# DoHoonKim8/halo2-lasso

Measured on AMD Instinct MI355X. Metric: lasso_prove_time_ms, lower is better.
Workload: dtype u256 (BN254 Fr/Fq, 8x u32 Montgomery); 1 GPU; 2^24 AND Lasso lookup (32-bit operands, 4 chunks of 8+8 bits); lookups_per_proof=16777216, pcs=multilinear KZG (BN254), proof_bytes=64256, parallelism=1 GPU

## Files before the change

### bindings/rust/src/sys.rs

```rust
#![allow(non_camel_case_types, dead_code)]
use halo2_curves::bn256::{Fr, G1Affine, G2Affine};
use std::os::raw::{c_char, c_int, c_void};

pub type lh_status = c_int;
pub const LH_OK: lh_status = 0;
pub const LH_ERR_INVALID_SUMCHECK: lh_status = -1;
pub const LH_ERR_INVALID_PCS_PARAM: lh_status = -2;
pub const LH_ERR_INVALID_PCS_OPEN: lh_status = -3;
pub const LH_ERR_INVALID_SNARK: lh_status = -4;
pub const LH_ERR_SERIALIZATION: lh_status = -5;
pub const LH_ERR_TRANSCRIPT: lh_status = -6;
pub const LH_ERR_DEVICE: lh_status = -7;
pub const LH_ERR_ARG: lh_status = -8;

pub const LH_SC_MAX_TERMS: usize = 48;
pub const LH_SC_MAX_FACTORS: usize = 4;
pub const LH_SC_EVALUATIONS: c_int = 0;
pub const LH_SC_COEFFICIENTS: c_int = 1;
pub const LH_LASSO_MAX_CHUNKS: usize = 8;
pub const LH_LASSO_MAX_MEMORIES: usize = 16;
pub const LH_LASSO_MAX_TERMS: usize = 16;
pub const LH_RCCL_UNIQUE_ID_BYTES: usize = 128;

#[repr(C)] pub struct lh_ctx { _p: [u8; 0] }
// ... 71 lines not shown
    pub g_num_factors: [u8; LH_LASSO_MAX_TERMS],
    pub g_factor: [[u8; LH_SC_MAX_FACTORS]; LH_LASSO_MAX_TERMS],
}

#[repr(C)]
pub struct lh_comm {
    pub rank: c_int,
    pub size: c_int,
    pub user: *mut c_void,
    pub all_gather: Option<unsafe extern "C" fn(*mut c_void, *const c_void, *mut c_void, usize) -> c_int>,
    pub all_gather_device: Option<unsafe extern "C" fn(*mut c_void, *const c_void, *mut c_void, usize, *mut c_void) -> c_int>,
}

#[repr(C)]
pub struct lh_hp_lookup { pub inputs: *const lh_expr, pub tables: *const lh_expr, pub width: usize }
#[repr(C)] #[derive(Clone, Copy)]
pub struct lh_hp_lasso_lookup {
    pub table: lh_lasso_table,
    pub output_poly: usize,
    pub chunk_polys: [usize; LH_LASSO_MAX_CHUNKS],
}
#[repr(C)]
pub struct lh_hp_param {
    pub num_vars: usize,
    pub num_instance_polys: usize,
    pub num_instances: *const usize,
    pub num_preprocess_polys: usize,
    pub d_preprocess_polys: *const *const c_void,
    pub num_witness_polys: usize,
    pub num_challenges: usize,
    pub num_lookups: usize,
    pub lookups: *const lh_hp_lookup,
    pub num_permutation_polys: usize,
    pub permutation_poly_index: *const usize,
    pub d_permutation_polys: *const *const c_void,
    pub num_permutation_z_polys: usize,
    pub expression: lh_expr,
    pub num_lasso_lookups: usize,
    pub lasso_lookups: *const lh_hp_lasso_lookup,
}
#[repr(C)]
pub struct lh_hp_vparam {
    pub num_vars: usize,
    pub num_instance_polys: usize,
    pub num_instances: *const usize,
    pub num_witness_polys: usize,
    pub num_challenges: usize,
    pub num_lookups: usize,
    pub num_permutation_z_polys: usize,
    pub expression: lh_expr,
    pub num_preprocess_polys: usize,
    pub preprocess_comms: *const G1Affine,
    pub num_permutation_polys: usize,
    pub permutation_comms: *const G1Affine,
    pub num_lasso_lookups: usize,
    pub lasso_lookups: *const lh_hp_lasso_lookup,
}
#[repr(C)]
pub struct lh_hp_circuit {
    pub user: *mut c_void,
    pub synthesize: Option<unsafe extern "C" fn(*mut c_void, usize, *const Fr, usize, *mut *const c_void, usize) -> c_int>,
}

#[repr(C)]
#[derive(Clone, Copy, Debug, Default)]
pub struct lh_lasso_route {
    pub open_small_depth: u32,
    pub open_small_passes: u32,
    pub eq_factored_rounds: u32,
    pub standard_rounds: u32,
    pub rw_leaf_rounds: u32,
    pub resident_tails: u32,
    pub resident_rounds: u32,
    pub packed_ts_pairs: u32,
    pub derived_commitments: u32,
    pub sorted_dim_reuse: u32,
    pub sharded_rounds: u32,
    pub shard_exchanges: u32,
    pub window_table_jobs: u32,
    pub open_precommit: u32,
    pub resident_layers: u32,
    pub pp_folds: u32,
    pub msm_half_batches: u32,
    pub reserved: [u32; 7],
}

extern "C" {
    pub fn lh_last_error() -> *const c_char;
    pub fn lh_version() -> *const c_char;
    pub fn lh_ctx_create(device_id: c_int, out: *mut *mut lh_ctx) -> lh_status;
    pub fn lh_ctx_destroy(ctx: *mut lh_ctx);
    pub fn lh_ctx_sync(ctx: *mut lh_ctx) -> lh_status;
    pub fn lh_ctx_stream(ctx: *mut lh_ctx) -> *mut c_void;
    pub fn lh_alloc(ctx: *mut lh_ctx, bytes: usize, d_out: *mut *mut c_void) -> lh_status;
    pub fn lh_free(ctx: *mut lh_ctx, d_ptr: *mut c_void) -> lh_status;
    pub fn lh_upload(ctx: *mut lh_ctx, d_dst: *mut c_void, src: *const c_void, bytes: usize) -> lh_status;
    pub fn lh_download(ctx: *mut lh_ctx, dst: *mut c_void, d_src: *const c_void, bytes: usize) -> lh_status;
    pub fn lh_fr_from_u64(ctx: *mut lh_ctx, d_in: *const u64, n: usize, d_out: *mut Fr) -> lh_status;
    pub fn lh_fr_from_u32(ctx: *mut lh_ctx, d_in: *const u32, n: usize, d_out: *mut Fr) -> lh_status;
    pub fn lh_fr_batch_invert(ctx: *mut lh_ctx, d_in: *const Fr, n: usize, d_out: *mut Fr) -> lh_status;
    pub fn lh_fix_var(ctx: *mut lh_ctx, d_in: *const Fr, n_in: usize, x: *const Fr, d_out: *mut Fr) -> lh_status;
    pub fn lh_eq_xy(ctx: *mut lh_ctx, y: *const Fr, num_vars: usize, d_out: *mut Fr) -> lh_status;
    pub fn lh_evaluate(ctx: *mut lh_ctx, d_polys: *const *const Fr, num_polys: usize, num_vars: usize,
                       point: *const Fr, out_evals: *mut Fr) -> lh_status;
    pub fn lh_lincomb(ctx: *mut lh_ctx, d_polys: *const *const Fr, w: *const Fr, num_polys: usize, n: usize,
                      d_out: *mut Fr) -> lh_status;
    pub fn lh_sumcheck_prove(ctx: *mut lh_ctx, prover_kind: c_int, num_vars: usize, expr: *const lh_sop,
                             d_polys: *const *const Fr, num_polys: usize, ys: *const Fr, num_ys: usize,
                             sum: *const Fr, t: *mut lh_transcript, out_challenges: *mut Fr, out_evals: *mut Fr) -> lh_status;
    pub fn lh_sumcheck_prove_expr(ctx: *mut lh_ctx, num_vars: usize, expr: *const lh_expr, d_polys: *const *const Fr,
                                  num_polys: usize, challenges: *const Fr, num_challenges: usize, ys: *const Fr,
                                  num_ys: usize, sum: *const Fr, t: *mut lh_transcript, out_challenges: *mut Fr,
                                  out_evals: *mut Fr) -> lh_status;
    pub fn lh_sumcheck_verify(prover_kind: c_int, num_vars: usize, degree: usize, sum: *const Fr,
                              t: *mut lh_transcript, out_eval: *mut Fr, out_x: *mut Fr) -> lh_status;
    pub fn lh_gkr_fractional_prove(ctx: *mut lh_ctx, num_batching: usize, num_vars: usize,
                                   claimed_p_0s: *const *const Fr, claimed_q_0s: *const *const Fr,
                                   d_ps: *const *const Fr, d_qs: *const *const Fr, t: *mut lh_transcript,
                                   out_p_xs: *mut Fr, out_q_xs: *mut Fr, out_x: *mut Fr) -> lh_status;
    pub fn lh_msm(ctx: *mut lh_ctx, d_scalars: *const Fr, d_bases: *const G1Affine, n: usize, out: *mut G1Affine) -> lh_status;
    pub fn lh_msm_u32(ctx: *mut lh_ctx, d_scalars: *const u32, d_bases: *const G1Affine, n: usize, out: *mut G1Affine) -> lh_status;
    pub fn lh_srs_upload(ctx: *mut lh_ctx, eqs_flat: *const G1Affine, num_vars: usize, out: *mut *mut lh_srs) -> lh_status;
    pub fn lh_srs_num_vars(srs: *const lh_srs) -> usize;
    pub fn lh_srs_free(ctx: *mut lh_ctx, srs: *mut lh_srs);
    pub fn lh_mkzg_batch_commit(ctx: *mut lh_ctx, srs: *const lh_srs, d_polys: *const *const Fr, num_polys: usize,
                                num_vars: usize, out_comms: *mut G1Affine) -> lh_status;
    pub fn lh_mkzg_open(ctx: *mut lh_ctx, srs: *const lh_srs, d_poly: *const Fr, num_vars: usize, point: *const Fr,
                        t: *mut lh_transcript, out_eval: *mut Fr) -> lh_status;
    pub fn lh_mkzg_batch_open(ctx: *mut lh_ctx, srs: *const lh_srs, num_vars: usize, d_polys: *const *const Fr,
                              num_polys: usize, points: *const Fr, num_points: usize, evals: *const lh_evaluation,
                              num_evals: usize, t: *mut lh_transcript) -> lh_status;
    pub fn lh_mkzg_vp_new(g1: *const G1Affine, g2: *const G2Affine, ss: *const G2Affine, num_vars: usize,
                          out: *mut *mut lh_mkzg_vp) -> lh_status;
    pub fn lh_mkzg_vp_free(vp: *mut lh_mkzg_vp);
    pub fn lh_mkzg_verify(vp: *const lh_mkzg_vp, comm: *const G1Affine, point: *const Fr, num_vars: usize,
                          eval: *const Fr, t: *mut lh_transcript) -> lh_status;
    pub fn lh_mkzg_batch_verify(vp: *const lh_mkzg_vp, num_vars: usize, comms: *const G1Affine, num_comms: usize,
                                points: *const Fr, num_points: usize, evals: *const lh_evaluation, num_evals: usize,
                                t: *mut lh_transcript) -> lh_status;
    pub fn lh_lasso_prove(ctx: *mut lh_ctx, srs: *const lh_srs, table: *const lh_lasso_table, num_vars: usize,
                          d_dims: *const *const u32, t: *mut lh_transcript) -> lh_status;
    pub fn lh_lasso_verify(vp: *const lh_mkzg_vp, table: *const lh_lasso_table, num_vars: usize,
                           t: *mut lh_transcript) -> lh_status;
    pub fn lh_ctx_set_comm(ctx: *mut lh_ctx, comm: *const lh_comm, shard_bit: usize) -> lh_status;
    pub fn lh_rccl_unique_id(out: *mut u8) -> lh_status;
    pub fn lh_ctx_set_comm_rccl(ctx: *mut lh_ctx, rank: c_int, size: c_int, unique_id: *const u8, shard_bit: usize) -> lh_status;
    pub fn lh_ctx_set_comm_loopback(ctx: *mut lh_ctx, rank: c_int, size: c_int, shard_bit: usize) -> lh_status;
    pub fn lh_ctx_comm_stats(ctx: *mut lh_ctx, out: *mut u64) -> lh_status;
    pub fn lh_ctx_comm_phase_stats(ctx: *mut lh_ctx, out: *mut u64, reset: c_int) -> lh_status;
    pub fn lh_ctx_memory_stats(ctx: *mut lh_ctx, out: *mut u64) -> lh_status;
    pub fn lh_ctx_host_cpus(ctx: *mut lh_ctx, bus_id: *mut c_char, bus_id_cap: usize, cpulist: *mut c_char, cpulist_cap: usize) -> lh_status;
    pub fn lh_shard_extract(ctx: *mut lh_ctx, d_global: *const c_void, n_local: usize, shard_bit: usize, rho: usize,
                            rank: usize, elem_bytes: usize, d_local: *mut c_void) -> lh_status;
    pub fn lh_ctx_set_option(ctx: *mut lh_ctx, name: *const c_char, value: i64) -> lh_status;
    pub fn lh_ctx_get_option(ctx: *mut lh_ctx, name: *const c_char, out: *mut i64) -> lh_status;
    pub fn lh_lasso_last_route(ctx: *mut lh_ctx, out: *mut lh_lasso_route) -> lh_status;
    pub fn lh_lasso_prove_sharded(ctx: *mut lh_ctx, srs: *const lh_srs, table: *const lh_lasso_table, num_vars: usize,
                                  d_dims_local: *const *const u32, t: *mut lh_transcript) -> lh_status;
    pub fn lh_hyperplonk_prove(ctx: *mut lh_ctx, srs: *const lh_srs, pp: *const lh_hp_param,
                               instances: *const *const Fr, d_witness_polys: *const *const Fr,
                               t: *mut lh_transcript) -> lh_status;
    pub fn lh_hyperplonk_prove_sharded(ctx: *mut lh_ctx, srs: *const lh_srs, pp: *const lh_hp_param,
                                       instances: *const *const Fr, d_witness_polys_local: *const *const Fr,
                                       t: *mut lh_transcript) -> lh_status;
    pub fn lh_hyperplonk_prove_phases(ctx: *mut lh_ctx, srs: *const lh_srs, pp: *const lh_hp_param, num_phases: usize,
                                      num_witness_polys: *const usize, num_challenges: *const usize,
                                      instances: *const *const Fr, circuit: *const lh_hp_circuit,
// ... 135 lines not shown
```

### halo2-lasso_amd/__init__.py

```python
import ctypes as C

from . import _ffi
from ._ffi import (lh_fr, lh_g1, lh_sop, lh_evaluation, lh_lasso_table, lh_transcript,
                   LH_SC_EVALUATIONS, LH_SC_COEFFICIENTS)

R_MOD = 0x30644E72E131A029B85045B68181585D2833E84879B9709143E1F593F0000001
Q_MOD = 0x30644E72E131A029B85045B68181585D97816A916871CA8D3C208C16D87CFD47
_MONT = 1 << 256
_MONT_INV_R = pow(_MONT, -1, R_MOD)
_MONT_INV_Q = pow(_MONT, -1, Q_MOD)

SUBTABLE_IDENTITY, SUBTABLE_AND, SUBTABLE_XOR = 0, 1, 2


class Error(Exception):
    code = None


class InvalidSumcheck(Error):
    code = _ffi.LH_ERR_INVALID_SUMCHECK


class InvalidPcsParam(Error):
    code = _ffi.LH_ERR_INVALID_PCS_PARAM
# ... 1360 lines not shown
                return _ffi.LH_ERR_ARG
            C.memmove(recv, out, len(out))
            return 0
        except Exception:
            return _ffi.LH_ERR_DEVICE
    comm = _ffi.lh_comm()
    comm.rank, comm.size, comm.user = rank, size, None
    comm.all_gather = _ffi._AG_CB(cb)
    ctx._comm_keepalive = (comm, cb)
    _check(ctx.lib.lh_ctx_set_comm(ctx.h, C.byref(comm), shard_bit))


def rccl_unique_id():
    buf = C.create_string_buffer(_ffi.LH_RCCL_UNIQUE_ID_BYTES)
    _check(_ffi.load().lh_rccl_unique_id(buf))
    return buf.raw


def attach_comm_rccl(ctx, rank, size, unique_id, shard_bit):
    if len(unique_id) != _ffi.LH_RCCL_UNIQUE_ID_BYTES:
        raise ArgumentError("unique id must be %d bytes" % _ffi.LH_RCCL_UNIQUE_ID_BYTES)
    _check(ctx.lib.lh_ctx_set_comm_rccl(ctx.h, rank, size, unique_id, shard_bit))


def comm_stats(ctx):
    out = (C.c_uint64 * 2)()
    _check(ctx.lib.lh_ctx_comm_stats(ctx.h, out))
    return {"device": int(out[0]), "host": int(out[1])}


def comm_phase_stats(ctx, reset=False):
    out = (C.c_uint64 * 16)()
    _check(ctx.lib.lh_ctx_comm_phase_stats(ctx.h, out, 1 if reset else 0))
    names = ["witness", "commit", "surge", "leaves", "gkr", "evals", "open", "outside"]
    return {nm: {"collectives": int(out[2 * i]), "bytes": int(out[2 * i + 1])} for i, nm in enumerate(names) if out[2 * i]}


def memory_stats(ctx):
    out = (C.c_uint64 * 4)()
    _check(ctx.lib.lh_ctx_memory_stats(ctx.h, out))
    return {"arena_high_water_bytes": int(out[0]), "arena_reserved_bytes": int(out[1]), "device_free_bytes": int(out[2]),
            "device_total_bytes": int(out[3])}


def attach_comm_loopback(ctx, rank, size, shard_bit):
    _check(ctx.lib.lh_ctx_set_comm_loopback(ctx.h, rank, size, shard_bit))


def detach_comm(ctx):
    _check(ctx.lib.lh_ctx_set_comm(ctx.h, None, 0))
    ctx._comm_keepalive = None


def shard_of(column, rank, size, shard_bit):
    rho = size.bit_length() - 1
    n = len(column)
    return column.reshape(n >> (shard_bit + rho), size, 1 << shard_bit)[:, rank, :].reshape(-1).copy()


def shard_poly(poly, rank, size, shard_bit):
    rho = size.bit_length() - 1
    n_local = (1 << poly.num_vars) >> rho
    out = poly.ctx.alloc(32 * n_local)
    _check(poly.ctx.lib.lh_shard_extract(poly.ctx.h, poly.ptr, n_local, shard_bit, rho, rank, 32, out.ptr))
    return MultilinearPolynomial(poly.ctx, out, poly.num_vars - rho)


def lasso_prove_sharded(pp, table, num_vars, dims_local, transcript):
    if len(dims_local) != table.c:
        raise ArgumentError("expected %d dim columns" % table.c)
    t = table.to_c()
    _check(pp.ctx.lib.lh_lasso_prove_sharded(pp.ctx.h, pp.h, C.byref(t), num_vars, _ptr_array(dims_local), transcript.p))


def lasso_last_timing(ctx):
    out = (C.c_double * _ffi.LH_LASSO_NUM_PHASES)()
    _check(ctx.lib.lh_lasso_last_timing(ctx.h, out))
    names = ["witness", "commit", "surge", "leaves", "gkr", "evals", "open_n", "open_l", "total"]
    return dict(zip(names, list(out)))


ROUTE_FIELDS = ["open_small_depth", "open_small_passes", "eq_factored_rounds", "standard_rounds", "rw_leaf_rounds",
                "resident_tails", "resident_rounds", "packed_ts_pairs", "derived_commitments", "sorted_dim_reuse",
                "sharded_rounds", "shard_exchanges", "window_table_jobs", "open_precommit", "resident_layers", "pp_folds", "msm_half_batches"]


def lasso_last_route(ctx):
    out = (C.c_uint32 * 24)()
    _check(ctx.lib.lh_lasso_last_route(ctx.h, out))
    return dict(zip(ROUTE_FIELDS, [int(v) for v in out]))


def set_option(ctx, name, value):
    _check(ctx.lib.lh_ctx_set_option(ctx.h, name.encode(), int(value)))


def get_option(ctx, name):
    out = C.c_int64(0)
    _check(ctx.lib.lh_ctx_get_option(ctx.h, name.encode(), C.byref(out)))
    return int(out.value)


def profile_enable(ctx, on=True):
    _check(ctx.lib.lh_profile_enable(ctx.h, int(on)))


def profile_read(ctx):
    n = C.c_size_t()
    _check(ctx.lib.lh_profile_read(ctx.h, None, 0, C.byref(n)))
    arr = (_ffi.lh_prof_rec * max(n.value, 1))()
    _check(ctx.lib.lh_profile_read(ctx.h, arr, n.value, C.byref(n)))
    return [dict(name=r.name.decode(), ms=r.ms, bytes=r.bytes, muls=r.muls, items=r.items) for r in arr[:n.value]]


from . import expression
```

### halo2-lasso_amd/csrc/dev.cpp

```cpp
#include <string.h>
#include <stdlib.h>
#include <ctype.h>
#include <errno.h>
#include <sched.h>
#include <atomic>
#include <condition_variable>
#include <mutex>
#include <thread>
#include <functional>
#include <memory>
#include <emmintrin.h>
#include <hip/hip_ext.h>
#include <vector>
#include <chrono>
#include "dev.hpp"

namespace lh {

static thread_local std::string g_last_error;
void set_last_error(const char* msg) { g_last_error = msg ? msg : ""; }
const char* get_last_error() { return g_last_error.c_str(); }

Arena::~Arena() {
  for (auto& b : blocks_) (void)hipFree(b.p);
}

void* Arena::alloc(size_t bytes) {
  bytes = (bytes + 255) & ~(size_t)255;
  if (bytes == 0) bytes = 256;
  return alloc_raw(bytes);
}
void* Arena::alloc_raw(size_t bytes) {
  while (true) {
    if (!blocks_.empty()) {
      Block& b = blocks_[cur_];
      if (b.used + bytes <= b.size) {
        void* p = b.p + b.used;
        b.used += bytes;
        size_t tot = 0;
        for (size_t i = 0; i <= cur_; i++) tot += blocks_[i].used;
        if (tot > high_) high_ = tot;
        return p;
      }
      if (cur_ + 1 < blocks_.size()) {
        cur_++;
        blocks_[cur_].used = 0;
        continue;
      }
    }
    size_t want = blocks_.empty() ? ((size_t)64 << 20) : blocks_.back().size * 2;
    if (want < bytes) want = bytes;
    void* p = nullptr;
    LH_HIP(hipMalloc(&p, want));
    blocks_.push_back(Block{(char*)p, want, 0});
    cur_ = blocks_.size() - 1;
  }
}

void Arena::release(Mark m) {
  if (blocks_.empty()) return;
  for (size_t i = m.block + 1; i < blocks_.size(); i++) blocks_[i].used = 0;
  cur_ = m.block;
  blocks_[cur_].used = m.used;
}

void Ctx::opt_in_lds(const void* fn, int bytes) {
  for (const void* f : lds_opted)
    if (f == fn) return;
  LH_HIP(hipFuncSetAttribute(fn, hipFuncAttributeMaxDynamicSharedMemorySize, bytes));
  lds_opted.push_back(fn);
}

static const struct {
  const char* name;
  int64_t Options::*field;
  int64_t lo, hi;
} OPTION_TABLE[] = {
    {"open_small_min_vars", &Options::open_small_min_vars, 0, 64}, {"open_small_depth", &Options::open_small_depth, 0, 2},
    {"sc_eq_factoring", &Options::sc_eq_factoring, 0, 1},          {"lasso_pack_ts", &Options::lasso_pack_ts, 0, 1},
    {"sc_tail", &Options::sc_tail, 0, 1},                          {"sc_tail_max_len", &Options::sc_tail_max_len, 0, (int64_t)1 << 20},
    {"shard_exchange_log", &Options::shard_exchange_log, 0, 40},   {"msm_window_tables", &Options::msm_window_tables, 0, 40},
    {"open_precommit", &Options::open_precommit, 0, 64},           {"gkr_resident", &Options::gkr_resident, 0, 1},
    {"sc_pp_fold", &Options::sc_pp_fold, 0, 2},                    {"msm_half_batches", &Options::msm_half_batches, 0, 1},
    {"comm_round", &Options::comm_round, 0, 2},
};

int64_t* Options::find(const char* name) {
  if (!name) return nullptr;
  for (const auto& o : OPTION_TABLE)
    if (strcmp(o.name, name) == 0) return &(this->*o.field);
  return nullptr;
}
bool Options::in_range(const char* name, int64_t value) {
  if (!name) return false;
  for (const auto& o : OPTION_TABLE)
    if (strcmp(o.name, name) == 0) return value >= o.lo && value <= o.hi;
  return false;
}

static bool env_number(const char* name, bool real, double lo, double hi, double& out, std::atomic<bool>* said = nullptr) {
  const char* e = getenv(name);
  if (!e || !*e) return false;
  char* end = nullptr;
  errno = 0;
  const double v = real ? strtod(e, &end) : (double)strtoll(e, &end, 10);
  if (end != e && *end == 0 && errno == 0 && v >= lo && v <= hi) {
    out = v;
    return true;
  }
  if (!said || !said->exchange(true))
    fprintf(stderr, "[lasso-hip] %s=%s is outside [%lld, %lld]: ignored\n", name, e, (long long)lo, (long long)hi);
  return false;
}

Options::Options() {
  for (const auto& o : OPTION_TABLE) {
    std::string env = "LH_";
    for (const char* p = o.name; *p; p++) env.push_back((char)toupper((unsigned char)*p));
    double v;
    if (!env_number(env.c_str(), false, (double)o.lo, (double)o.hi, v)) continue;
    this->*o.field = (int64_t)v;
    if (o.field == &Options::open_small_min_vars) open_small_min_vars_forced = true;
  }
}

enum KnobKind { INT, REAL, WORD, PATH };
static constexpr struct KnobRow {
  const char* env;
  KnobKind kind;
  double dflt, lo, hi;
  bool live;
  const char* word;
} KNOB_TABLE[] = {
    {"LH_SC_TAIL_G", INT, 0, 0, 1024},
    {"LH_MSM_C_OFF", INT, 4, -32, 32},
    {"LH_MSM_C_MAX", INT, 17, 1, 31},
    {"LH_MSM_K2", INT, 4, 2, 64},
    {"LH_MSM_SEG", INT, 0, 0, 256},
    {"LH_MSM_SLAB_LOG", INT, 16, 0, 31},
    {"LH_MSM_TREE_MAX", INT, 262144, 0, 1 << 30},
    {"LH_MSM_QUAD_MAX", INT, 262144, 0, 1 << 30},
    {"LH_MSM_TWO_LEVEL", INT, 1, 0, 1},
    {"LH_MSM_HALF_MIN_LOG", INT, 24, 0, 63},
    {"LH_MSM_HALF_COVER", INT, 12, 0, 1 << 20},
    {"LH_EXPR_MONOMIALS", INT, 0, 0, 1},
    {"LH_EXPR_JIT_MIN_VARS", INT, 16, 0, 64},
    {"LH_EXPR_EF_MIN_VARS", INT, 14, 2, 64},
    {"LH_FIN_LANES_MIN_BYTES", REAL, 0, -1, 1e18},
    {"LH_SC_U32", INT, 1, 0, 1}, {"LH_OPEN_U32_ROUNDS", INT, 1, 0, 1}, {"LH_OPEN_FOLD_COLS", INT, 1, 0, 1},
    {"LH_HOST_THREADS", INT, 48, 0, 4096},
    {"LH_JIT_CACHE", INT, 1, 0, 1}, {"LH_JIT_CACHE_DIR", PATH, 0, 0, 0},
    {"LH_EXPR_JIT", INT, 1, 0, 1},
    {"LH_SC_TAIL_TIMEOUT_MS", REAL, 2000, 0, 1e7, true}, {"LH_GKR_START_TIMEOUT_MS", REAL, 25, 0, 1e7, true},
    {"LH_COMM_WAIT_TIMEOUT_MS", INT, 30000, 1, 1e9}, {"LH_COMM_A2A", WORD, 0, 0, 1, false, "allgather"},
    {"LH_COMM_PROBE", INT, 1, 0, 1},
    {"LH_HOST_TRACE", INT, 0, 0, 1, true}, {"LH_SC_TAIL_TRACE", INT, 0, 0, 1}, {"LH_GKR_TRACE", INT, 0, 0, 1},
    {"LH_SC_DEBUG", INT, 0, 0, 1}, {"LH_MSM_DEBUG", INT, 0, 0, 1}, {"LH_HP_DEBUG", INT, 0, 0, 1}, {"LH_COMM_DEBUG", INT, 0, 0, 1},
    {"LH_OPEN_SMALL_CHECK", INT, 0, 0, 1},
    {"LH_COMM_A2A_SELF", INT, 0, 0, 1}, {"LH_COMM_PROBE_FAIL", INT, 0, 0, 1}, {"LH_SHARDED_COUNTERS_MIN_R", INT, 2, 1, 1 << 20},
};
static_assert(sizeof(KNOB_TABLE) / sizeof(KNOB_TABLE[0]) == (size_t)Knob::COUNT, "KNOB_TABLE: one row per Knob");

static double knob_read(const KnobRow& r, std::atomic<bool>* said) {
  double v = r.dflt;
  if (r.kind != WORD) {
    env_number(r.env, r.kind == REAL, r.lo, r.hi, v, said);
  } else if (const char* e = getenv(r.env)) {
// ... 417 lines not shown
```

### halo2-lasso_amd/csrc/dev.hpp

```cpp
#pragma once
#include <hip/hip_runtime_api.h>
#include <stdint.h>
#include <stdarg.h>
#include <stdio.h>
#include <functional>
#include <string>
#include <vector>
#include <utility>
#include <stdexcept>

#include "../../include/lasso_hip.h"
#include "ec.cuh"

namespace lh {

struct Error : std::exception {
  int code;
  std::string msg;
  Error(int c, std::string m) : code(c), msg(std::move(m)) {}
  const char* what() const noexcept override { return msg.c_str(); }
};

void set_last_error(const char* msg);

// ... 1 lines not shown
  do {                                                                                     \
    hipError_t e_ = (expr);                                                                \
    if (e_ != hipSuccess)                                                                  \
      throw ::lh::Error(LH_ERR_DEVICE, std::string(#expr) + ": " + hipGetErrorString(e_)); \
  } while (0)

#define LH_REQUIRE(cond, code, text) \
  do {                               \
    if (!(cond)) throw ::lh::Error((code), (text)); \
  } while (0)

class Arena {
 public:
  struct Mark {
    size_t block, used;
  };
  ~Arena();
  void* alloc(size_t bytes);
  void* alloc_raw(size_t bytes);
  template <class T>
  T* alloc_n(size_t n) {
    return (T*)alloc(n * sizeof(T));
  }
  Mark mark() const { return {cur_, blocks_.empty() ? 0 : blocks_[cur_].used}; }
  void release(Mark m);
  size_t high_water() const { return high_; }
  size_t reserved() const {
    size_t t = 0;
    for (const Block& b : blocks_) t += b.size;
    return t;
  }

 private:
  struct Block {
    char* p;
    size_t size, used;
  };
  std::vector<Block> blocks_;
  size_t cur_ = 0, high_ = 0;
};

struct ArenaScope {
  Arena& a;
  Arena::Mark m;
  explicit ArenaScope(Arena& a_) : a(a_), m(a_.mark()) {}
  ~ArenaScope() { a.release(m); }
};

struct ProfRec {
  char name[40];
  double ms;
  double bytes;
  double muls;
  double items;
};

struct ScFinishArgs {
  uint32_t* ticket;
  uint32_t last_ticket;
  Fr* out_host;
  uint32_t* flag;
  uint32_t seq;
  uint64_t* wide;
  uint32_t tag;
  uint64_t* lanes;
};
constexpr uint32_t FIN_LANE_SUMS = 65536;
constexpr unsigned SC_LANE_TAG_SHIFT = 40;

struct Options {
  int64_t open_small_min_vars = 21;
  bool open_small_min_vars_forced = false;
  int64_t open_small_depth = 0;
  int64_t sc_eq_factoring = 1;
  int64_t lasso_pack_ts = 1;
  int64_t sc_tail = 1;
  int64_t sc_tail_max_len = 8192;
  int64_t shard_exchange_log = 19;
  int64_t open_precommit = 1;
  int64_t msm_window_tables = 0;
  int64_t sc_pp_fold = 1;
  int64_t msm_half_batches = 1;
  int64_t gkr_resident = 1;
  int64_t comm_round = 0;
  Options();
  int64_t* find(const char* name);
  static bool in_range(const char* name, int64_t value);
};

enum class Knob {
  SC_TAIL_G, MSM_C_OFF, MSM_C_MAX, MSM_K2, MSM_SEG, MSM_SLAB_LOG, MSM_TREE_MAX, MSM_QUAD_MAX, MSM_TWO_LEVEL, MSM_HALF_MIN_LOG,
  MSM_HALF_COVER, EXPR_MONOMIALS, EXPR_JIT_MIN_VARS, EXPR_EF_MIN_VARS,
  FIN_LANES_MIN_BYTES, SC_U32, OPEN_U32_ROUNDS, OPEN_FOLD_COLS,
  HOST_THREADS, JIT_CACHE, JIT_CACHE_DIR, EXPR_JIT, SC_TAIL_TIMEOUT_MS, GKR_START_TIMEOUT_MS, COMM_WAIT_TIMEOUT_MS, COMM_A2A,
  COMM_PROBE,
  HOST_TRACE, SC_TAIL_TRACE, GKR_TRACE, SC_DEBUG, MSM_DEBUG, HP_DEBUG, COMM_DEBUG, OPEN_SMALL_CHECK,
  COMM_A2A_SELF, COMM_PROBE_FAIL, SHARDED_COUNTERS_MIN_R,
  COUNT
};
double knob(Knob k);
const char* knob_text(Knob k);
struct RouteStats {
  uint32_t v[LH_LASSO_ROUTE_WORDS] = {0};
  enum { OPEN_DEPTH, OPEN_PASSES, EF_ROUNDS, STD_ROUNDS, RW_ROUNDS, TAILS, TAIL_ROUNDS, PACKED_TS, DERIVED, SORTED_REUSE,
         SHARDED_ROUNDS, SHARD_EXCHANGES, WIN_TABLE_JOBS, OPEN_PRECOMMIT, RESIDENT_LAYERS, PP_FOLDS, MSM_HALF_BATCHES };
};

class HostWorker {
 public:
  HostWorker();
  ~HostWorker();
  void submit(std::function<void()> fn);
  void wait();
 private:
  struct Impl;
  Impl* impl_;
};

struct OpenPrecommit;
struct Ctx {
  Options opt;
  RouteStats route;
  int device = 0;
  hipStream_t stream = nullptr;
  Arena arena;
  void* pinned = nullptr;
  size_t pinned_bytes = 0;
  int num_cus = 256;
  int wall_clock_khz = 100000;
  double lasso_ms[LH_LASSO_NUM_PHASES] = {0};
  lh_comm comm = {0, 1, nullptr, nullptr, nullptr};
  bool has_comm = false;
  bool comm_loopback = false;
  size_t shard_bit = 0;
  bool shard_active = false;
  void* rccl_comm = nullptr;
  void* comm_stage = nullptr;
  size_t comm_stage_bytes = 0;
  uint64_t comm_stats[2] = {0, 0};
  uint64_t comm_phase_stats[8][2] = {};
  int comm_phase = 7;
  Fr* sc_redirect = nullptr;
  uint64_t* sc_wide = nullptr;
  uint32_t sc_tag = 0;
  uint32_t sc_tag_seq = 0;
  uint64_t* lanes_host = nullptr;
  bool comm_host_recv_ok = true;
  Fr* round_out(Fr* out_host) const { return sc_redirect ? sc_redirect : out_host; }
  void wait_round(uint32_t seq) {
    if (!sc_redirect) wait_flag(seq);
  }
  uint64_t* tail_trace = nullptr;
  std::vector<std::pair<const char*, double>> host_stamps;
  bool host_trace_on = false;
  void host_stamp(const char* tag);
  void host_stamps_print();
  struct EqHalfEntry {
    std::vector<uint8_t> key;
    const Fr* table;
    bool sharded = false;
  };
  std::vector<EqHalfEntry> eq_half_cache;
  bool prof = false;
  std::vector<ProfRec> prof_recs;
  bool live = false;
  struct LiveRec {
    ProfRec rec;
    hipEvent_t e0, e1;
    uint32_t batch;
  };
  std::vector<LiveRec> live_recs;
  std::vector<hipEvent_t> live_pool;
  uint32_t live_batch = 0;
  hipEvent_t live_event();
  void live_resolve(std::vector<ProfRec>& out);
  bool is_helper = false;
  Ctx* helper = nullptr;
  lh_ctx* helper_handle = nullptr;
  OpenPrecommit* precommit = nullptr;
  HostWorker* worker = nullptr;
  hipEvent_t handoff_ev = nullptr;
  hipEvent_t phase_ev[LH_LASSO_NUM_PHASES] = {};
  bool phase_ev_pending = false;
  void phase_times_resolve();
  hipEvent_t prof_ev[2] = {nullptr, nullptr};
  void* pin(size_t bytes);
  void* stage = nullptr;
  size_t stage_bytes = 0;
// ... 126 lines not shown
void k_lincomb_bind2(Ctx&, const uint32_t* const* cols, const size_t* lens, const Fr* w, size_t count, const Fr& r0, const Fr& r1,
                     const Fr* eq_level, size_t size, Fr* out, Fr* out_host);
void k_sc_round_u32_bind2(Ctx&, const uint32_t* col, const Fr* eq_level, const Fr& r0, const Fr& r1, size_t size, Fr* out,
                          Fr* out_host);
void k_lincomb_mixed(Ctx&, const Fr* const* fr, const Fr* wfr, size_t num_fr, const uint32_t* const* sm,
                     const size_t* sm_len, const Fr* wsm, size_t num_sm, size_t n, Fr* out);
void k_tree_up(Ctx&, const Fr* in, size_t half, Fr* out);
void k_tree_up_multi(Ctx&, const Fr* const* in, Fr* const* out, size_t count, size_t half);
void k_tree_tops(Ctx&, const Fr* const* in, Fr* const* out, const int* H, size_t count);
void k_frac_up(Ctx&, const Fr* p, const Fr* q, size_t half, Fr* vp, Fr* vq);
void k_quotient_step(Ctx&, const Fr* rem, size_t half, const Fr& x, Fr* q, Fr* rem_out);
void k_lasso_rw_leaves(Ctx&, const uint32_t* dim, const uint32_t* e, const uint32_t* ts, size_t n,
                       const Fr& gamma, const Fr& gamma2, const Fr& tau, Fr* rs, Fr* ws);
void k_lasso_rw_leaves_up(Ctx&, const uint32_t* dim, const uint32_t* e, const uint32_t* ts, size_t n, const Fr& gamma,
                          const Fr& gamma2, const Fr& tau, Fr* rs, Fr* ws, Fr* rs_up, Fr* ws_up);
void k_lasso_if_leaves(Ctx&, int subtable, uint32_t chunk_bits, const uint32_t* final_cts, size_t m,
                       const Fr& gamma, const Fr& gamma2, const Fr& tau, Fr* init, Fr* fin);
void k_or_u32(Ctx&, const uint32_t* const* cols, size_t count, size_t n, uint32_t* out_host);
void k_fill_u32(Ctx&, uint32_t* out, uint32_t value, size_t n);
void k_pack_u32(Ctx&, const uint32_t* a, const uint32_t* b, uint32_t shift, size_t n, uint32_t* out);
void k_delta_u32(Ctx&, const uint32_t* col, size_t len, size_t half, uint64_t offset, uint32_t* out_lo, uint32_t* out_hi);
void k_lasso_counters(Ctx&, const uint32_t* const* dims, size_t cc, size_t n, size_t m, uint32_t* const* read_ts,
                      uint32_t* const* final_cts, uint32_t* const* keep_sorted = nullptr, uint32_t* const* keep_index = nullptr);
void k_cs_partition(Ctx&, const uint32_t* const* dims, size_t cc, size_t n, size_t m, unsigned rho, unsigned j, unsigned hi_bits,
                    uint32_t* const* sidx, uint32_t* const* send, uint32_t* start_host, bool* bad_out);
void k_cs_rank(Ctx&, const uint32_t* const* recv, const size_t* n_recv, size_t cc, unsigned hi_bits, unsigned a_bits, size_t m_loc,
               uint32_t* const* ret, uint32_t* counts);
void k_cs_scatter(Ctx&, const uint32_t* const* back, const uint32_t* const* sidx, size_t cc, size_t n, uint32_t* const* read_ts);
void k_cs_final(Ctx&, const uint32_t* all_counts, size_t cc, size_t m, unsigned rho, size_t m_loc, uint32_t* const* final_cts);
void k_lasso_subtable_read(Ctx&, int subtable, uint32_t chunk_bits, const uint32_t* dim, size_t n, uint32_t* e);
struct LassoG {
  uint32_t num_terms;
  Fr coeff[LH_LASSO_MAX_TERMS];
  uint8_t nfac[LH_LASSO_MAX_TERMS];
  uint8_t fac[LH_LASSO_MAX_TERMS][LH_SC_MAX_FACTORS];
  const uint32_t* e[LH_LASSO_MAX_MEMORIES];
};
void k_lasso_output(Ctx&, const LassoG& g, size_t n, Fr* a);
struct LassoGSmall {
  uint32_t num_terms;
  uint32_t coeff[LH_LASSO_MAX_TERMS];
  uint8_t fac[LH_LASSO_MAX_TERMS];
  const uint32_t* e[LH_LASSO_MAX_MEMORIES];
};
void k_lasso_output_small(Ctx&, const LassoGSmall& g, size_t n, uint32_t* a);
bool k_fr_to_index(Ctx&, const Fr* in, size_t n, uint32_t bits, uint32_t* out);
bool k_fr_tables_equal(Ctx&, const Fr* a, const Fr* b, size_t n);

void rccl_unique_id(uint8_t out[LH_RCCL_UNIQUE_ID_BYTES]);
void comm_attach_rccl(Ctx&, int rank, int size, const uint8_t id[LH_RCCL_UNIQUE_ID_BYTES], size_t shard_bit);
void comm_probe_host_recv(Ctx&);
void comm_attach_loopback(Ctx&, int rank, int size, size_t shard_bit);
void comm_detach(Ctx&);
void comm_all_gather_dev(Ctx&, const void* d_send, void* d_recv, size_t bytes);
void comm_all_gather_host(Ctx&, const void* send, void* recv, size_t bytes);
void comm_all_to_all_multi(Ctx&, size_t nbuf, const void* const* d_send, const size_t* send_off, const size_t* send_cnt,
                           void* const* d_recv, const size_t* recv_off, const size_t* recv_cnt, const size_t* peer_off,
                           const void* send_base, size_t send_stride, size_t elem);
void comm_sum_publish(Ctx&, const Fr* d_part, Fr* d_scratch, size_t count, Fr* out_host, uint32_t seq);
void comm_sum_lanes(Ctx&, uint64_t* d_lanes, uint64_t* d_scratch, size_t count, Fr* out_host);
uint32_t comm_next_tag(Ctx&);
void k_loopback_allreduce_lanes(Ctx&, const uint64_t* d_in, size_t n, size_t R, uint64_t* out);

void k_shard_merge(Ctx&, const void* gathered, size_t n_local, size_t j, size_t rho, size_t elem, void* global);
void k_gather_interleave(Ctx&, const Fr* gathered, size_t count, size_t n_local, size_t R, size_t block, Fr* const* out);
void k_sum_publish(Ctx&, const Fr* all, size_t R, size_t D, Fr* out_host, uint32_t seq);
void k_shard_extract(Ctx&, const void* global, size_t n_local, size_t j, size_t rho, size_t s, size_t elem, void* local);
void k_loopback_gather(Ctx&, const void* d_send, void* d_recv, size_t bytes, size_t R);
void k_scale(Ctx&, const Fr* in, const Fr& w, size_t n, Fr* out);

constexpr int SC_MAX_TABLES = 72;
struct ScRound {
  const Fr* in[SC_MAX_TABLES];
  Fr* out[SC_MAX_TABLES];
  uint32_t num_tables;
  uint32_t num_terms;
  int32_t global_eq;
  Fr coeff[LH_SC_MAX_TERMS];
  uint8_t coeff_is_one[LH_SC_MAX_TERMS];
  uint8_t nfac[LH_SC_MAX_TERMS];
  uint8_t fac[LH_SC_MAX_TERMS][LH_SC_MAX_FACTORS];
  Fr r;
  const Fr* eq_level;
  uint8_t pp;
};
bool k_sc_round(Ctx&, const ScRound& rd, int degree, bool bind, size_t size, Fr* evals_host);
bool k_sc_round_streams(const ScRound& rd, int degree, size_t size);
void k_eq_levels(Ctx&, const Fr* in, size_t n_in, Fr* const* levels, size_t nlev);
constexpr int SC_OPEN_MAX_TERMS = 6;
struct ScOpenRound {
  const Fr* in[SC_OPEN_MAX_TERMS];
  Fr* out[SC_OPEN_MAX_TERMS];
  const Fr* eq_level[SC_OPEN_MAX_TERMS];
  uint32_t num_terms;
  Fr r;
};
void k_sc_round_open(Ctx&, const ScOpenRound& rd, bool bind, size_t size, Fr* out_host);

constexpr int SC_RW_MAX_PAIRS = 8;
struct ScRwRound {
  const Fr* l[SC_RW_MAX_PAIRS];
  const Fr* r[SC_RW_MAX_PAIRS];
  Fr* lo[SC_RW_MAX_PAIRS];
  Fr* ro[SC_RW_MAX_PAIRS];
  Fr cs[SC_RW_MAX_PAIRS], k[SC_RW_MAX_PAIRS];
  const Fr* eq_level;
  Fr rchal;
  uint32_t num_pairs;
};
void k_sc_round_rw(Ctx&, const ScRwRound& rd, bool bind, size_t size, Fr* out_host, bool fold = false);

struct TailChunk {
  uint32_t w[4];
};
struct TailMbox {
  TailChunk c[3];
  uint32_t pad[4];
};
constexpr uint32_t SC_TAIL_ABORT = 0xffffffffu;
constexpr int SC_TAIL_MAX_DEGREE = 6;
size_t k_sc_tail_capacity(const Ctx&, const ScRound& rd, int degree);
void k_sc_tail_launch(Ctx&, const ScRound& rd, int degree, size_t n0, bool first_bind, size_t num_out, uint32_t seq0,
                      TailChunk* msg_host, Fr* out_host);
void k_sc_tail_resync(Ctx&);

constexpr int GKR_MAX_TREES = 16;
constexpr int GKR_MAX_VARS = 16;
constexpr uint32_t GKR_CAP = 128;
constexpr uint32_t GKR_THREADS = 256;
constexpr uint32_t GKR_MSG_CHUNKS = 3 * (GKR_MAX_TREES + GKR_MAX_VARS);
constexpr uint32_t GKR_START_FAILED = 0xfffffffeu;
enum { GKR_F_SPLIT = 1, GKR_F_BIND = 2, GKR_F_EQ = 4, GKR_F_NOMSG = 8, GKR_F_KOFF = 16 };
struct GkrLayerDev {
  const Fr* lv[GKR_MAX_TREES];
  const Fr* rv[GKR_MAX_TREES];
  uint32_t h, B;
  uint32_t g, s_log;
  uint32_t seq;
  uint32_t flags;
  const Fr* eq_level;
  Fr r_prev;
  Fr coef[GKR_MAX_TREES];
  Fr koff[GKR_MAX_TREES];
};
bool k_gkr_resident_geometry(uint32_t h, uint32_t* g, uint32_t* s_log);
void k_gkr_resident_launch(Ctx&, const GkrLayerDev* layers, size_t num_layers, TailChunk* msg_host, Fr* out_host);

struct ExtRound {
  const Fr* in[SC_MAX_TABLES];
  Fr* out[SC_MAX_TABLES];
  uint32_t num_tables, num_terms;
  const Fr* coeff;
  const uint8_t* is_one;
  const uint32_t* off;
  const uint8_t* fac;
  const uint8_t* store;
  Fr r;
};
void k_sc_round_ext(Ctx&, const ExtRound& rd, int degree, bool bind, size_t size, Fr* evals_host);
void k_rotate_gather(Ctx&, const Fr* poly, size_t num_vars, int rot, uint32_t primitive, uint32_t x_inv, Fr* out);
void k_identity_table(Ctx&, size_t n, Fr* out);
void k_identity_table_shard(Ctx&, size_t n_local, size_t j, size_t rho, size_t rank, Fr* out);
void k_bh_order(Ctx&, size_t num_vars, uint32_t primitive, uint32_t* order, uint32_t* nth);
void k_one_hot_table(Ctx&, size_t n, size_t hot, Fr* out);
enum { PROG_ADD = 0, PROG_SUB = 1, PROG_MUL = 2, PROG_NEG = 3, PROG_MOV = 4 };
enum { PROG_REG = 0, PROG_ATOM = 1, PROG_CONST = 2, PROG_PAIR = 3 };
constexpr int PROG_MAX_REGS = 8;
struct ProgRound {
  const Fr* in[SC_MAX_TABLES];
  uint32_t num_tables, num_instrs, num_regs, result_reg;
  const uint32_t* code;
  const Fr* consts;
};
struct JitKernel;
bool jit_enabled(size_t num_vars);
std::string jit_debug_source(const uint32_t* code, size_t num_instrs, uint32_t num_regs, uint32_t result_reg, int degree);
const JitKernel* jit_sc_round(const Ctx&, const uint32_t* host_code, size_t num_instrs, uint32_t num_regs, uint32_t result_reg, int degree);
unsigned jit_blocks_per_cu(const JitKernel*);
void jit_launch(Ctx&, const JitKernel*, const ProgRound& pr, unsigned points, unsigned grid, size_t size, Fr* partials, const ScFinishArgs& fin);
void k_sc_round_prog(Ctx&, const ProgRound& pr, int points, size_t size, Fr* evals_host, const JitKernel* jit = nullptr);
constexpr int LIN_MAX_TABLES = 8;
struct LinSums {
  const Fr* t[LIN_MAX_TABLES];
  Fr coeff[LIN_MAX_TABLES];
  uint32_t count;
};
void k_lin_sums(Ctx&, const LinSums& ls, size_t size, Fr* out_host);
enum { ROWS_ATOM_POLY = 0, ROWS_ATOM_IDENTITY = 1, ROWS_ATOM_LAGRANGE = 2 };
struct RowsAtom {
// ... 109 lines not shown
```

### halo2-lasso_amd/csrc/gkr.cpp

```cpp
#include <algorithm>
#include <functional>
#include <chrono>
#include <memory>
#include <thread>
#include "host.hpp"
#include "resident_host.hpp"

namespace lh {

FracSumCheckResult prove_fractional_sum_check(Ctx& c, size_t B, size_t num_vars, const HFr* const* claimed_p_0s,
                                              const HFr* const* claimed_q_0s, const Fr* const* d_ps,
                                              const Fr* const* d_qs, Transcript& tr) {
  LH_REQUIRE(B != 0, LH_ERR_ARG, "fractional sum-check: num_batching == 0");
  LH_REQUIRE(num_vars >= 1, LH_ERR_ARG, "fractional sum-check: num_vars == 0");
  LH_REQUIRE(3 * B <= LH_SC_MAX_TERMS && 4 * B + 1 <= (size_t)SC_MAX_TABLES, LH_ERR_ARG,
             "fractional sum-check: too many fractions for one round kernel");
  ArenaScope scope(c.arena);
  std::vector<std::vector<const Fr*>> lp(num_vars), lq(num_vars);
  for (size_t b = 0; b < B; b++) {
    lp[0].push_back(d_ps[b]);
    lq[0].push_back(d_qs[b]);
  }
  for (size_t h = 1; h < num_vars; h++) {
    size_t half = (size_t)1 << (num_vars - h);
// ... 107 lines not shown
    std::vector<int> top_H(B);
    std::vector<size_t> cur_h(B);
    size_t max_h = 0;
    for (size_t b = 0; b < B; b++) {
      level[b].resize(num_vars[b]);
      level[b][num_vars[b] - 1] = d_leaves[b];
      size_t h = num_vars[b] - 1;
      if (d_level_up && d_level_up[b] && h > SMALL && (!sh.on || sh.sharded(h))) {
        level[b][h - 1] = d_level_up[b];
        h--;
      }
      cur_h[b] = h;
      max_h = std::max(max_h, h);
    }
    for (size_t h = max_h; h >= 1 && (h > SMALL || sh.sharded(h + 1)); h--) {
      std::vector<const Fr*> ins;
      std::vector<Fr*> outs;
      std::vector<size_t> who;
      const bool in_sh = sh.sharded(h + 1), out_sh = sh.sharded(h);
      const size_t half = (size_t)1 << (in_sh ? h - sh.rho : h);
      for (size_t b = 0; b < B; b++) {
        if (cur_h[b] != h) continue;
        ins.push_back(level[b][h]);
        who.push_back(b);
        cur_h[b] = h - 1;
      }
      if (ins.empty()) continue;
      if (in_sh && !out_sh) {
        Fr* block = c.arena.alloc_n<Fr>(ins.size() * half);
        std::vector<Fr*> rep(ins.size());
        for (size_t k = 0; k < ins.size(); k++) {
          outs.push_back(block + k * half);
          rep[k] = c.arena.alloc_n<Fr>((size_t)1 << h);
        }
        k_tree_up_multi(c, ins.data(), outs.data(), ins.size(), half);
        comm_gather_tables(c, block, ins.size(), half, half, rep.data());
        c.route.v[RouteStats::SHARD_EXCHANGES]++;
        for (size_t k = 0; k < ins.size(); k++) level[who[k]][h - 1] = rep[k];
      } else {
        for (size_t k = 0; k < ins.size(); k++) {
          outs.push_back(c.arena.alloc_n<Fr>(half));
          level[who[k]][h - 1] = outs.back();
        }
        k_tree_up_multi(c, ins.data(), outs.data(), ins.size(), half);
      }
    }
    for (size_t b = 0; b < B; b++) {
      const size_t h = cur_h[b];
      LH_REQUIRE(h <= SMALL && !sh.sharded(h + 1), LH_ERR_ARG, "grand product: internal level mismatch");
      Fr* tops = c.arena.alloc_n<Fr>(((size_t)2 << h));
      top_in[b] = level[b][h];
      top_out[b] = tops;
      top_H[b] = (int)h;
      for (size_t k = 0; k < h; k++) level[b][k] = tops + (((size_t)2 << k) - 2);
    }
    k_tree_tops(c, top_in.data(), top_out.data(), top_H.data(), B);
  }
  std::vector<HFr> top(2 * B);
  {
    std::vector<const Fr*> heads;
    for (size_t b = 0; b < B; b++) heads.push_back(level[b][0]);
    Fr* out = (Fr*)c.pin(2 * SC_MAX_TABLES * sizeof(Fr));
    k_gather_heads(c, heads.data(), heads.size(), 2, out);
    memcpy(top.data(), out, 2 * B * sizeof(Fr));
  }
  GrandProductResult res;
  res.roots.resize(B);
  res.claims.resize(B);
  res.points.resize(B);
  for (size_t b = 0; b < B; b++) res.roots[b] = top[2 * b] * top[2 * b + 1];
  tr.write_field_elements(res.roots);

  std::vector<HFr> claims = res.roots, y;
  HFr resident_lam;
  bool have_resident_lam = false;
  GkrResident resident(c);
  std::vector<GkrLayerDev> resident_layers;
  if (c.opt.gkr_resident && c.opt.sc_tail && c.opt.sc_eq_factoring) {
    std::vector<GkrLayerDev> layers;
    for (size_t h = 1; h < max_depth; h++) {
      GkrLayerDev L;
      memset(&L, 0, sizeof(L));
      uint32_t nb = 0;
      bool ok = !sh.sharded(h + 1) && k_gkr_resident_geometry((uint32_t)h, &L.g, &L.s_log);
      bool any_leaf = false, all_leaf = true;
      for (size_t b = 0; b < B && ok; b++) {
        if (num_vars[b] <= h) continue;
        ok = nb < (uint32_t)GKR_MAX_TREES && level[b][h] != nullptr;
        if (!ok) break;
        any_leaf = any_leaf || num_vars[b] == h + 1;
        all_leaf = all_leaf && num_vars[b] == h + 1;
        L.lv[nb++] = level[b][h];
      }
      if (ok && plus_one && any_leaf && all_leaf) ok = false;
      if (!ok || nb == 0) break;
      L.h = (uint32_t)h, L.B = nb;
      layers.push_back(L);
    }
    resident_layers.swap(layers);
  }
  if (trees_built) trees_built();
  if (!resident_layers.empty()) resident.launch(resident_layers);
  for (size_t h = 0; h < max_depth; h++) {
    std::vector<size_t> active;
    for (size_t b = 0; b < B; b++)
      if (num_vars[b] > h) active.push_back(b);
    if (h >= 1 && resident.live && h <= resident.H) {
      HFr lam = tr.squeeze_challenge();
      HFr claim = HFr::zero(), power = HFr::one();
      std::vector<HFr> coeff;
      for (size_t b : active) {
        claim += claims[b] * power;
        coeff.push_back(power);
        power *= lam;
      }
      std::vector<HFr> x, evals;
      if (resident.layer(h, coeff, y, claim, tr, x, evals)) {
        c.route.v[RouteStats::RESIDENT_LAYERS]++;
        tr.write_field_elements(evals);
        HFr mu = tr.squeeze_challenge();
        x.push_back(mu);
        y = x;
        for (size_t k = 0; k < active.size(); k++) {
          const size_t b = active[k];
          const HFr &l = evals[2 * k], &r = evals[2 * k + 1];
          claims[b] = l + mu * (r - l);
          if (num_vars[b] == h + 1) {
            res.claims[b] = claims[b];
            res.points[b] = y;
          }
        }
        continue;
      }
      resident_lam = lam, have_resident_lam = true;
    }
    const bool layer_sh = sh.sharded(h + 1);
    const size_t half = (size_t)1 << (layer_sh ? h - sh.rho : h);
    std::vector<HFr> x, evals;
    if (h == 0) {
      for (size_t b : active) {
        evals.push_back(top[2 * b]);
        evals.push_back(top[2 * b + 1]);
      }
    } else {
      HFr lam = have_resident_lam ? resident_lam : tr.squeeze_challenge();
      have_resident_lam = false;
      HFr claim = HFr::zero(), power = HFr::one();
      lh_sop expr;
      memset(&expr, 0, sizeof(expr));
      expr.global_eq = 0;
      std::vector<const Fr*> polys;
      ScOptions so;
      so.sum_is_exact = true, so.sharded = layer_sh;
      bool pairs = plus_one != nullptr && active.size() % 2 == 0 && active.size() / 2 <= (size_t)SC_RW_MAX_PAIRS;
      for (size_t k = 0; k < active.size() && pairs; k++) {
        const size_t b = active[k];
        pairs = num_vars[b] == h + 1 && (k % 2 == 0 ? !plus_one[b] : (plus_one[b] && active[k - 1] + 1 == b));
      }
      if (pairs) {
        const size_t P = active.size() / 2;
        ScRwPairs rw;
        rw.num_pairs = (uint32_t)P;
        rw.const_total = HFr::zero();
        HFr cw_sum = HFr::zero();
        bool degenerate = false;
        uint32_t t = 0;
        for (size_t i = 0; i < P; i++) {
// ... 66 lines not shown
```

### halo2-lasso_amd/csrc/host.hpp

```cpp
#pragma once
#include <string.h>
#include <functional>
#include <map>
#include <mutex>
#include <vector>
#include "dev.hpp"
#include "ff_host.hpp"

namespace lh {

const char* get_last_error();

typedef host::Fr HFr;
typedef host::G1Affine HG1;

static inline Fr dev(const HFr& f) {
  Fr r;
  memcpy(&r, &f, 32);
  return r;
}
static inline HFr hst(const Fr& f) {
  HFr r;
  memcpy(&r, &f, 32);
  return r;
// ... 48 lines not shown
  }
  void common_commitment(const HG1& p) { check(t->common_commitment(t->user, (const lh_g1*)&p)); }
  HFr read_field_element() {
    LH_REQUIRE(t->read_field_element, LH_ERR_ARG, "transcript cannot read (write-only callback table)");
    HFr f;
    check(t->read_field_element(t->user, (lh_fr*)&f));
    return f;
  }
  std::vector<HFr> read_field_elements(size_t n) {
    std::vector<HFr> v(n);
    for (auto& f : v) f = read_field_element();
    return v;
  }
  HG1 read_commitment() {
    LH_REQUIRE(t->read_commitment, LH_ERR_ARG, "transcript cannot read (write-only callback table)");
    HG1 p;
    check(t->read_commitment(t->user, (lh_g1*)&p));
    return p;
  }
  std::vector<HG1> read_commitments(size_t n) {
    std::vector<HG1> v(n);
    for (auto& p : v) p = read_commitment();
    return v;
  }
};

typedef std::function<void(size_t num_vars, const HG1* comms, size_t num_comms, const HFr* points, size_t num_points,
                           const lh_evaluation* evals, size_t num_evals, Transcript& tr)>
    PcsBatchVerify;

std::vector<HFr> host_eq_xy(const std::vector<HFr>& y);
HFr host_eq_xy_eval(const HFr* x, const HFr* y, size_t n);
std::vector<HFr> evaluate_polys(Ctx&, const Fr* const* d_polys, size_t count, size_t num_vars, const HFr* point);

struct SumCheckResult {
  std::vector<HFr> challenges;
  std::vector<HFr> evals;
  bool u32_terms_built = false;
};
struct ScRwPairs {
  uint32_t num_pairs;
  HFr cs[SC_RW_MAX_PAIRS], k[SC_RW_MAX_PAIRS];
  HFr const_total;
};
struct ScU32 {
  const uint32_t* col = nullptr;
  bool have_sums = false;
  Fr odd, s2, s3;
};
struct ScU32Terms {
  struct Poly {
    std::vector<const uint32_t*> col;
    std::vector<size_t> len;
    std::vector<Fr> w;
  };
  std::vector<Poly> polys;
};
struct ScOptions {
  bool sum_is_exact = false;
  bool sharded = false;
  const ScRwPairs* rw = nullptr;
  const ScU32* u32 = nullptr;
  const ScU32Terms* u32_terms = nullptr;
};
SumCheckResult sum_check_prove(Ctx&, int prover_kind, size_t num_vars, const lh_sop& expr, const Fr* const* d_polys,
                               size_t num_polys, const HFr* ys, size_t num_ys, const HFr& sum, Transcript& tr,
                               const ScOptions& opt = ScOptions());

const Fr* eq_half_lookup(Ctx&, const HFr* y, size_t num_vars, bool sharded = false);
const Fr* eq_half_get(Ctx&, const HFr* y, size_t num_vars, bool sharded = false);
struct EqHalfScope {
  Ctx& c;
  size_t mark;
  explicit EqHalfScope(Ctx& c_) : c(c_), mark(c_.eq_half_cache.size()) {}
  ~EqHalfScope() { c.eq_half_cache.resize(mark); }
};

typedef std::function<void(const Fr* const*, Fr* const*, const Fr&, bool, size_t, Fr*)> RoundFn;
struct EqFactoring {
  struct One {
    size_t table;
    const HFr* y;
    std::vector<const Fr*> level;
    HFr S, S_prev;
    std::vector<HFr> q;
  };
  std::vector<One> eqs;
  bool per_term = false;
  bool trusted_claim = false;
  bool untrusted = false;
  std::vector<HFr> inv_1my;
  HFr c;
  HFr add_const;
  HFr kappa = HFr::one(), lin0 = HFr::zero(), lin1 = HFr::zero();
  std::function<bool(bool bind, size_t size)> streams;
  std::function<void(const Fr* const* in, Fr* const* out, const Fr& r, bool bind, size_t size, size_t round, int points,
                     Fr* out_host)>
      round;
  std::function<bool(const std::vector<const Fr*>& cur, bool bind, const HFr& r_prev, size_t n0, size_t round, const HFr& claim,
                     Transcript& tr, SumCheckResult& res)>
      resident_tail;
};
SumCheckResult sum_check_loop(Ctx&, int prover_kind, size_t num_vars, int degree, std::vector<const Fr*> cur,
                              const std::vector<char>& used, size_t num_polys, const HFr& sum, Transcript& tr,
                              bool sharded, const RoundFn& round_fn, const ScRound* tail_rd = nullptr,
                              EqFactoring* ef = nullptr);
SumCheckResult sum_check_prove_expr(Ctx&, size_t num_vars, const lh_expr& expr, const Fr* const* d_polys,
                                    size_t num_polys, const HFr* challenges, size_t num_challenges, const HFr* ys,
                                    size_t num_ys, const HFr& sum, Transcript& tr, bool sharded = false);

std::vector<HFr> evaluate_polys(Ctx&, const Fr* const* d_polys, size_t count, size_t num_vars, const HFr* point, bool sharded);
void comm_sum_fr(Ctx&, HFr* v, size_t n);
void comm_sum_points(Ctx&, HG1* pts, size_t n);
void comm_gather_tables(Ctx&, const Fr* local_block, size_t count, size_t n_local, size_t block, Fr* const* out);
void comm_gather_concat(Ctx&, const Fr* local, size_t n_local, Fr* out);
void eq_xy_shard(Ctx&, const Shard&, const HFr* y, size_t num_vars, size_t first, Fr* out_local);

struct FracSumCheckResult {
  std::vector<HFr> p_xs, q_xs, x;
};
FracSumCheckResult prove_fractional_sum_check(Ctx&, size_t num_batching, size_t num_vars,
                                              const HFr* const* claimed_p_0s, const HFr* const* claimed_q_0s,
                                              const Fr* const* d_ps, const Fr* const* d_qs, Transcript& tr);
struct GrandProductResult {
  std::vector<HFr> roots, claims;
  std::vector<std::vector<HFr>> points;
};
GrandProductResult prove_grand_product(Ctx&, size_t num_trees, const Fr* const* d_leaves, const size_t* num_vars,
                                       Transcript& tr, const Fr* const* d_level_up = nullptr,
                                       const uint8_t* plus_one = nullptr,
                                       const std::function<void()>& trees_built = nullptr);

struct Srs {
  G1Affine* d_eqs = nullptr;
  size_t num_vars = 0;
  const G1Affine* eq(size_t k) const { return d_eqs + (((size_t)1 << k) - 1); }
  mutable std::vector<G1Affine*> shard_levels;
  mutable int shard_rank = -1;
  mutable size_t shard_R = 0, shard_j = 0;
  mutable std::map<size_t, HG1> level_sums;
  mutable std::map<size_t, HG1> shard_level_sums;
  struct WinTable {
    G1Affine* d = nullptr;
    uint32_t c = 0, W = 0;
  };
  mutable std::map<size_t, WinTable> win_tables;
};
const Srs::WinTable* srs_window_table(Ctx&, const Srs&, size_t level);
const G1Affine* srs_shard_level(Ctx&, const Srs&, size_t level);
Srs* mkzg_setup(Ctx&, const HFr* ss, size_t num_vars);
std::vector<HG1> mkzg_batch_commit(Ctx&, const Srs&, const Fr* const* d_polys, size_t num_polys, size_t num_vars);
std::vector<HG1> mkzg_batch_commit_u32(Ctx&, const Srs&, const uint32_t* const* d_polys, size_t num_polys,
                                       size_t num_vars);
struct SmallOpen;
HFr mkzg_open(Ctx&, const Srs&, const Fr* d_poly, size_t num_vars, const HFr* point, Transcript& tr,
              const SmallOpen* small = nullptr);
struct SmallLinear {
  std::vector<size_t> poly;
  std::vector<HFr> coeff;
};
struct SmallPoly {
  const uint32_t* ptr = nullptr;
  size_t len = 0;
  uint32_t bits = 0;
  const SmallLinear* linear = nullptr;
};
// ... 229 lines not shown
```

### halo2-lasso_amd/csrc/kernels_poly.hip

```cpp
#include <hip/hip_runtime.h>
#include <string.h>
#include <algorithm>
#include "dev.hpp"
#include "ff_host.hpp"
#include "reduce.cuh"
#include "resident.cuh"
#include "wide.cuh"

namespace lh {

static inline dim3 grid_for(size_t n, int block = 256, size_t cap = 4096) {
  size_t g = (n + block - 1) / block;
  if (g < 1) g = 1;
  if (g > cap) g = cap;
  return dim3((unsigned)g);
}
#define GSTRIDE(i, n) \
  for (size_t i = (size_t)blockIdx.x * blockDim.x + threadIdx.x; i < (n); i += (size_t)gridDim.x * blockDim.x)

__global__ void fr_from_u64_kernel(const uint64_t* __restrict__ in, size_t n, Fr* __restrict__ out) {
  GSTRIDE(i, n) out[i] = from_u64<FrParams>(in[i]);
}
__global__ void fr_from_u32_kernel(const uint32_t* __restrict__ in, size_t n, Fr* __restrict__ out) {
  GSTRIDE(i, n) out[i] = from_u64<FrParams>(in[i]);
// ... 156 lines not shown
  int total = (int)count * k;
  hipLaunchKernelGGL(gather_heads_kernel, dim3((total + 63) / 64), dim3(64), 0, c.stream, p, (int)count, k, out_host);
  c.sync();
}

__global__ void eq_expand_kernel(const Fr* __restrict__ cur, size_t n_cur, Fr y, Fr* __restrict__ nxt) {
  GSTRIDE(k, n_cur) {
    Fr e = cur[k];
    Fr hi = mul(e, y);
    nxt[2 * k + 1] = hi;
    nxt[2 * k] = sub(e, hi);
  }
}
__global__ void fr_set_one_kernel(Fr* p) { p[0] = Fr::one(); }

constexpr int EQ_SMALL = 9;
__global__ void eq_outer_kernel(const Fr* __restrict__ lo_tab, int lo_bits, const Fr* __restrict__ hi_tab, size_t n,
                                Fr* __restrict__ out) {
  const size_t mask = ((size_t)1 << lo_bits) - 1;
  GSTRIDE(i, n) out[i] = mul(hi_tab[i >> lo_bits], lo_tab[i & mask]);
}

constexpr int EQ_GROUPS = 4;
struct EqGroups {
  Fr y[EQ_GROUPS][EQ_SMALL];
  int levels[EQ_GROUPS];
  Fr* out[EQ_GROUPS];
};
__global__ __launch_bounds__(256) void eq_groups_kernel(EqGroups g) {
  __shared__ Fr a[1 << EQ_SMALL];
  __shared__ Fr b[1 << (EQ_SMALL - 1)];
  const int levels = g.levels[blockIdx.x];
  Fr* cur = (levels & 1) ? b : a;
  Fr* nxt = (levels & 1) ? a : b;
  if (threadIdx.x == 0) cur[0] = Fr::one();
  __syncthreads();
  int n = 1;
  for (int i = 0; i < levels; i++) {
    const Fr yi = g.y[blockIdx.x][i];
    for (int k = threadIdx.x; k < n; k += blockDim.x) {
      Fr e = cur[k];
      Fr hi = mul(e, yi);
      nxt[2 * k + 1] = hi;
      nxt[2 * k] = sub(e, hi);
    }
    __syncthreads();
    Fr* t = cur;
    cur = nxt;
    nxt = t;
    n <<= 1;
  }
  Fr* out = g.out[blockIdx.x];
  for (int k = threadIdx.x; k < n; k += blockDim.x) out[k] = cur[k];
}

void k_eq_xy(Ctx& c, const Fr* y, size_t num_vars, Fr* out) {
  ProfScope ps(c, "eq_xy", 64.0 * ((size_t)1 << num_vars), 1.0 * ((size_t)1 << num_vars), (double)((size_t)1 << num_vars));
  const size_t ngroups = std::max<size_t>(1, (num_vars + EQ_SMALL - 1) / EQ_SMALL);
  LH_REQUIRE(ngroups <= (size_t)EQ_GROUPS, LH_ERR_ARG, "eq_xy: too many variables");
  ArenaScope scope(c.arena);
  EqGroups g;
  size_t first[EQ_GROUPS], cnt[EQ_GROUPS];
  Fr* tab[EQ_GROUPS];
  for (size_t k = 0, done = 0; k < ngroups; k++) {
    cnt[k] = (num_vars - done + (ngroups - k) - 1) / (ngroups - k);
    first[k] = done;
    done += cnt[k];
    tab[k] = ngroups == 1 ? out : c.arena.alloc_n<Fr>((size_t)1 << cnt[k]);
    g.levels[k] = (int)cnt[k];
    g.out[k] = tab[k];
    for (size_t i = 0; i < cnt[k]; i++) g.y[k][i] = y[first[k] + cnt[k] - 1 - i];
  }
  hipLaunchKernelGGL(eq_groups_kernel, dim3((unsigned)ngroups), dim3(256), 0, c.stream, g);
  Fr* cur = tab[0];
  size_t done = cnt[0];
  for (size_t k = 1; k < ngroups; k++) {
    const bool last = k + 1 == ngroups;
    const size_t n = (size_t)1 << (done + cnt[k]);
    Fr* dst = last ? out : c.arena.alloc_n<Fr>(n);
    hipLaunchKernelGGL(eq_outer_kernel, grid_for(n), 256, 0, c.stream, cur, (int)done, tab[k], n, dst);
    cur = dst;
    done += cnt[k];
  }
}

template <class T>
__global__ void shard_extract_kernel(const T* __restrict__ g, size_t n_local, unsigned j, unsigned rho, size_t s,
                                     T* __restrict__ local) {
  const size_t lo_mask = ((size_t)1 << j) - 1;
  GSTRIDE(i, n_local) local[i] = g[((i >> j) << (j + rho)) | (s << j) | (i & lo_mask)];
}
struct alignas(16) Bytes64 {
  uint4 a, b, c, d;
};
void k_shard_extract(Ctx& c, const void* global, size_t n_local, size_t j, size_t rho, size_t s, size_t elem,
                     void* local) {
  if (!n_local) return;
  dim3 g = grid_for(n_local);
  if (elem == 4)
    hipLaunchKernelGGL(shard_extract_kernel<uint32_t>, g, 256, 0, c.stream, (const uint32_t*)global, n_local, (unsigned)j,
                       (unsigned)rho, s, (uint32_t*)local);
  else if (elem == 32)
    hipLaunchKernelGGL(shard_extract_kernel<Fr>, g, 256, 0, c.stream, (const Fr*)global, n_local, (unsigned)j,
                       (unsigned)rho, s, (Fr*)local);
  else if (elem == 64)
    hipLaunchKernelGGL(shard_extract_kernel<Bytes64>, g, 256, 0, c.stream, (const Bytes64*)global, n_local, (unsigned)j,
                       (unsigned)rho, s, (Bytes64*)local);
  else
    throw Error(LH_ERR_ARG, "shard_extract: unsupported element size");
}
template <class T>
__global__ void shard_merge_kernel(const T* __restrict__ gathered, size_t n_local, unsigned j, unsigned rho,
                                   T* __restrict__ global) {
  const size_t lo_mask = ((size_t)1 << j) - 1, s_mask = ((size_t)1 << rho) - 1;
  GSTRIDE(g, n_local << rho) {
    const size_t s = (g >> j) & s_mask, local = ((g >> (j + rho)) << j) | (g & lo_mask);
    global[g] = gathered[s * n_local + local];
  }
}
void k_shard_merge(Ctx& c, const void* gathered, size_t n_local, size_t j, size_t rho, size_t elem, void* global) {
  if (!n_local) return;
  dim3 g = grid_for(n_local << rho);
  if (elem == 4)
    hipLaunchKernelGGL(shard_merge_kernel<uint32_t>, g, 256, 0, c.stream, (const uint32_t*)gathered, n_local, (unsigned)j,
                       (unsigned)rho, (uint32_t*)global);
  else if (elem == 32)
    hipLaunchKernelGGL(shard_merge_kernel<Fr>, g, 256, 0, c.stream, (const Fr*)gathered, n_local, (unsigned)j,
                       (unsigned)rho, (Fr*)global);
  else
    throw Error(LH_ERR_ARG, "shard_merge: unsupported element size");
}

struct InterleaveOut {
  Fr* out[SC_MAX_TABLES];
};
__global__ void gather_interleave_kernel(const Fr* __restrict__ gathered, unsigned count, size_t n_local, unsigned R,
                                         size_t block, InterleaveOut o) {
  const size_t full = n_local * R;
  GSTRIDE(e, full * count) {
    const size_t t = e / full, k = e % full, lo = k % block, q = k / block, hi = q / R, s = q % R;
    o.out[t][k] = gathered[((size_t)s * count + t) * n_local + hi * block + lo];
  }
}
void k_gather_interleave(Ctx& c, const Fr* gathered, size_t count, size_t n_local, size_t R, size_t block, Fr* const* out) {
  LH_REQUIRE(count <= (size_t)SC_MAX_TABLES, LH_ERR_ARG, "gather_interleave: too many tables");
  LH_REQUIRE(block >= 1 && n_local % block == 0, LH_ERR_ARG, "gather_interleave: bad block size");
  if (!count || !n_local) return;
  InterleaveOut o;
  for (size_t t = 0; t < count; t++) o.out[t] = out[t];
  hipLaunchKernelGGL(gather_interleave_kernel, grid_for(n_local * R * count), 256, 0, c.stream, gathered, (unsigned)count,
                     n_local, (unsigned)R, block, o);
}

__global__ void sum_publish_kernel(const Fr* __restrict__ all, unsigned R, unsigned D, Fr* __restrict__ out_host,
                                   uint32_t* flag, uint32_t seq) {
  if (threadIdx.x == 0) {
    for (unsigned x = 0; x < D; x++) {
      Fr acc = all[x];
      for (unsigned s = 1; s < R; s++) acc = add(acc, all[(size_t)s * D + x]);
      out_host[x] = acc;
    }
    __hip_atomic_store(flag, seq, __ATOMIC_RELEASE, __HIP_MEMORY_SCOPE_SYSTEM);
  }
}
void k_sum_publish(Ctx& c, const Fr* all, size_t R, size_t D, Fr* out_host, uint32_t seq) {
  hipLaunchKernelGGL(sum_publish_kernel, dim3(1), dim3(64), 0, c.stream, all, (unsigned)R, (unsigned)D, out_host, c.flag, seq);
// ... 1141 lines not shown
```

### halo2-lasso_amd/csrc/kernels_sumcheck.hip

```cpp
#include <hip/hip_runtime.h>
#include <stdlib.h>
#include <algorithm>
#include "dev.hpp"
#include "reduce.cuh"
#include "resident.cuh"

namespace lh {

struct ScArgs {
  ScRound rd;
  uint8_t store[LH_SC_MAX_TERMS][LH_SC_MAX_FACTORS];
};

template <bool BIND>
__device__ __forceinline__ void load_pair(const Fr* __restrict__ in, Fr* __restrict__ out, size_t b, const Fr& r,
                                          bool store, Fr& v0, Fr& v1) {
  if (BIND) {
    const Fr* p = in + 4 * b;
    Fr e0 = p[0], e1 = p[1], e2 = p[2], e3 = p[3];
    v0 = add(mul(sub(e1, e0), r), e0);
    v1 = add(mul(sub(e3, e2), r), e2);
    if (store) {
      out[2 * b] = v0;
      out[2 * b + 1] = v1;
    }
  } else {
    v0 = in[2 * b];
    v1 = in[2 * b + 1];
  }
}


typedef ScFinishArgs ScFinish;

template <int D>
__device__ __forceinline__ void finish_round(const ScFinish& f, const Fr* __restrict__ partials, Fr* lds) {
  __shared__ int is_last;
  if (!fin_ticket(f, &is_last)) return;
  const uint32_t blocks = gridDim.x;
#pragma unroll
  for (int x = 0; x < D; x++) {
    Fr acc = Fr::zero();
    for (uint32_t i = threadIdx.x; i < blocks; i += blockDim.x) acc = add(acc, fin_get(f, partials, (size_t)i * D + x));
    acc = block_reduce_sum(acc, lds);
    if (threadIdx.x == 0) f.out_host[x] = acc;
  }
  if (threadIdx.x == 0) publish_round(f, D);
}

template <int D, bool BIND>
__global__ __launch_bounds__(256) __attribute__((amdgpu_waves_per_eu(D <= 2 ? 4 : 1, D <= 2 ? 4 : 8))) void sc_round_kernel(ScArgs a, size_t size, uint32_t tp,
                                                       Fr* __restrict__ partials, ScFinish fin) {
  __shared__ Fr lds[4];
  const ScRound& rd = a.rd;
  Fr acc[D];
#pragma unroll
  for (int x = 0; x < D; x++) acc[x] = Fr::zero();

  const size_t items = size * tp;
  for (size_t w = (size_t)blockIdx.x * blockDim.x + threadIdx.x; w < items; w += (size_t)gridDim.x * blockDim.x) {
    const size_t b = tp == 1 ? w : w / tp;
    const uint32_t m_lo = tp == 1 ? 0u : (uint32_t)(w % tp);
    const uint32_t m_hi = tp == 1 ? rd.num_terms : m_lo + 1u;
    Fr s[D];
#pragma unroll
    for (int x = 0; x < D; x++) s[x] = Fr::zero();
    for (uint32_t m = m_lo; m < m_hi; m++) {
      Fr pm[D];
      const int nf = rd.nfac[m];
      if (nf == 0) {
#pragma unroll
        for (int x = 0; x < D; x++) pm[x] = rd.coeff_is_one[m] ? Fr::one() : rd.coeff[m];
      }
      for (int k = 0; k < nf; k++) {
        const int t = rd.fac[m][k];
        Fr v0, v1;
        load_pair<BIND>(rd.in[t], rd.out[t], b, rd.r, a.store[m][k] != 0, v0, v1);
        if (k == 0) {
          if (!rd.coeff_is_one[m]) {
            v0 = mul(v0, rd.coeff[m]);
            v1 = mul(v1, rd.coeff[m]);
          }
          Fr step = sub(v1, v0);
          pm[0] = v1;
#pragma unroll
          for (int x = 1; x < D; x++) pm[x] = add(pm[x - 1], step);
        } else {
          Fr step = sub(v1, v0);
          Fr val = v1;
          pm[0] = mul(pm[0], val);
#pragma unroll
          for (int x = 1; x < D; x++) {
            val = add(val, step);
            pm[x] = mul(pm[x], val);
          }
        }
      }
#pragma unroll
      for (int x = 0; x < D; x++) s[x] = add(s[x], pm[x]);
    }
    if (rd.eq_level) {
      const Fr e = rd.eq_level[b];
#pragma unroll
      for (int x = 0; x < D; x++) s[x] = mul(s[x], e);
    } else if (rd.global_eq >= 0) {
      Fr v0, v1;
      load_pair<BIND>(rd.in[rd.global_eq], rd.out[rd.global_eq], b, rd.r, m_lo == 0, v0, v1);
      Fr step = sub(v1, v0);
      Fr val = v1;
      s[0] = mul(s[0], val);
#pragma unroll
      for (int x = 1; x < D; x++) {
        val = add(val, step);
        s[x] = mul(s[x], val);
      }
    }
#pragma unroll
    for (int x = 0; x < D; x++) acc[x] = add(acc[x], s[x]);
  }
#pragma unroll
  for (int x = 0; x < D; x++) {
    Fr v = block_reduce_sum(acc[x], lds);
    if (threadIdx.x == 0) fin_put(fin, partials, (size_t)blockIdx.x * D + x, v);
  }
  if (gridDim.x == 1) {
    if (threadIdx.x == 0) publish_round(fin, D);
    return;
  }
  finish_round<D>(fin, partials, lds);
}

__device__ __forceinline__ Fr dpp_xor1(const Fr& v) {
  Fr o;
#pragma unroll
  for (int i = 0; i < 8; i++) o.l[i] = (uint32_t)__builtin_amdgcn_mov_dpp((int)v.l[i], 0xB1, 0xF, 0xF, true);
  return o;
}
template <bool BIND>
__device__ __forceinline__ Fr load_entry(const Fr* __restrict__ in, Fr* __restrict__ out, size_t i, const Fr& r, bool store) {
  if (BIND) {
    const Fr e0 = in[2 * i], e1 = in[2 * i + 1];
    const Fr v = add(mul(sub(e1, e0), r), e0);
    if (store) out[i] = v;
    return v;
  }
  return in[i];
}
__device__ __forceinline__ Fr at_lane_point(const Fr& v, bool odd) {
  const Fr o = dpp_xor1(v);
  return odd ? v : sub(dbl(o), v);
}
__device__ __forceinline__ void reduce_by_parity(const Fr& acc, bool odd, Fr* lds, Fr& even_sum, Fr& odd_sum) {
  even_sum = block_reduce_sum(odd ? Fr::zero() : acc, lds);
  odd_sum = block_reduce_sum(odd ? acc : Fr::zero(), lds);
}

template <bool BIND>
__global__ __launch_bounds__(256) void sc_round_e2_kernel(ScArgs a, size_t size, Fr* __restrict__ partials, ScFinish fin) {
  __shared__ Fr lds[4];
  const ScRound& rd = a.rd;
  Fr acc = Fr::zero();
  const size_t items = 2 * size;
  const bool odd = threadIdx.x & 1;
  for (size_t i = (size_t)blockIdx.x * blockDim.x + threadIdx.x; i < items; i += (size_t)gridDim.x * blockDim.x) {
    Fr s = Fr::zero();
    for (uint32_t m = 0; m < rd.num_terms; m++) {
      const int nf = rd.nfac[m];
      Fr pm = rd.coeff_is_one[m] ? Fr::one() : rd.coeff[m];
      for (int k = 0; k < nf; k++) {
        const int t = rd.fac[m][k];
        const Fr val = at_lane_point(load_entry<BIND>(rd.in[t], rd.out[t], i, rd.r, a.store[m][k] != 0), odd);
        pm = k == 0 ? (rd.coeff_is_one[m] ? val : mul(val, rd.coeff[m])) : mul(pm, val);
      }
      s = add(s, pm);
    }
    acc = add(acc, mul(s, rd.eq_level[i >> 1]));
  }
  Fr q2, q1;
  reduce_by_parity(acc, odd, lds, q2, q1);
  if (threadIdx.x == 0) {
    fin_put(fin, partials, (size_t)blockIdx.x * 2, q1);
    fin_put(fin, partials, (size_t)blockIdx.x * 2 + 1, q2);
  }
  if (gridDim.x == 1) {
    if (threadIdx.x == 0) publish_round(fin, 2);
    return;
  }
  finish_round<2>(fin, partials, lds);
}

template <bool BIND>
__global__ __launch_bounds__(256) __attribute__((amdgpu_waves_per_eu(3, 8))) void sc_round_pp_kernel(ScArgs a, size_t size, Fr* __restrict__ partials, ScFinish fin) {
  __shared__ Fr lds[4];
  const ScRound& rd = a.rd;
  Fr acc = Fr::zero();
  const size_t items = 2 * size;
  const bool odd = threadIdx.x & 1;
  const bool fold = BIND && rd.pp == 2;
  const uint32_t K = rd.num_terms;
  const Fr rch = rd.r;
  for (size_t i = (size_t)blockIdx.x * blockDim.x + threadIdx.x; i < items; i += (size_t)gridDim.x * blockDim.x) {
    Fr s = Fr::zero();
    for (uint32_t m0 = 0; m0 < K; m0 += 4) {
      Fr av[4], bv[4];
#pragma unroll
      for (int h2 = 0; h2 < 2; h2++) {
        const uint32_t ma = m0 + 2 * h2, mb = ma + 1;
        const bool va = ma < K, vb = mb < K;
        const int t0 = rd.fac[va ? ma : 0][0], t1 = rd.fac[va ? ma : 0][1], t2 = rd.fac[vb ? mb : 0][0], t3 = rd.fac[vb ? mb : 0][1];
        const Fr* __restrict__ p0 = rd.in[t0];
        const Fr* __restrict__ p1 = rd.in[t1];
        const Fr* __restrict__ p2 = rd.in[t2];
        const Fr* __restrict__ p3 = rd.in[t3];
        Fr x0, x1, x2, x3;
        if (BIND) {
          const Fr e00 = p0[2 * i], e01 = p0[2 * i + 1], e10 = p1[2 * i], e11 = p1[2 * i + 1];
          const Fr e20 = p2[2 * i], e21 = p2[2 * i + 1], e30 = p3[2 * i], e31 = p3[2 * i + 1];
          x0 = add(mul(sub(e01, e00), rch), e00);
          x1 = add(mul(sub(e11, e10), rch), e10);
          x2 = add(mul(sub(e21, e20), rch), e20);
          x3 = add(mul(sub(e31, e30), rch), e30);
        } else {
          x0 = p0[i], x1 = p1[i], x2 = p2[i], x3 = p3[i];
        }
        if (BIND && !fold) {
          if (va) rd.out[t0][i] = x0, rd.out[t1][i] = x1;
          if (vb) rd.out[t2][i] = x2, rd.out[t3][i] = x3;
        }
        if (va && !rd.coeff_is_one[ma]) x0 = mul(x0, rd.coeff[ma]);
        if (vb && !rd.coeff_is_one[mb]) x2 = mul(x2, rd.coeff[mb]);
        if (BIND && fold) {
          if (va) rd.out[t0][i] = x0, rd.out[t1][i] = x1;
          if (vb) rd.out[t2][i] = x2, rd.out[t3][i] = x3;
        }
        av[2 * h2] = va ? at_lane_point(x0, odd) : Fr::zero();
        bv[2 * h2] = va ? at_lane_point(x1, odd) : Fr::zero();
        av[2 * h2 + 1] = vb ? at_lane_point(x2, odd) : Fr::zero();
        bv[2 * h2 + 1] = vb ? at_lane_point(x3, odd) : Fr::zero();
      }
      s = add(s, dot<FrParams, 4>(av, bv));
    }
    acc = add(acc, mul(s, rd.eq_level[i >> 1]));
  }
  Fr q2, q1;
  reduce_by_parity(acc, odd, lds, q2, q1);
  if (threadIdx.x == 0) {
    fin_put(fin, partials, (size_t)blockIdx.x * 2, q1);
    fin_put(fin, partials, (size_t)blockIdx.x * 2 + 1, q2);
  }
  if (gridDim.x == 1) {
    if (threadIdx.x == 0) publish_round(fin, 2);
    return;
  }
  finish_round<2>(fin, partials, lds);
}

constexpr int LDS_VALS = 1280;
constexpr int LDS_ITEMS = 512;
struct ScLdsArgs {
  ScArgs a;
  uint8_t used[SC_MAX_TABLES];
  uint8_t slot_of[SC_MAX_TABLES];
  uint32_t num_used;
  uint32_t P;
  uint32_t vals_entries;
};

template <int D, bool BIND>
__global__ __launch_bounds__(256) void sc_round_lds_kernel(ScLdsArgs g, size_t size, Fr* __restrict__ partials,
                                                           ScFinish fin) {
  extern __shared__ __align__(16) unsigned char lds_raw[];
  const ScRound& rd = g.a.rd;
  const uint32_t P = g.P, U = g.num_used;
  Fr* vals = (Fr*)lds_raw;
  Fr* red = vals + g.vals_entries;
  const size_t b0 = (size_t)blockIdx.x * P;
  for (uint32_t e = threadIdx.x; e < U * P * 2; e += blockDim.x) {
    const uint32_t which = e & 1u, pl = (e >> 1) % P, u = (e >> 1) / P;
    const size_t b = b0 + pl;
    Fr v = Fr::zero();
    if (b < size) {
      const int t = g.used[u];
      if (BIND) {
        const Fr* p = rd.in[t] + 4 * b + 2 * which;
        Fr e0 = p[0], e1 = p[1];
        v = add(mul(sub(e1, e0), rd.r), e0);
        rd.out[t][2 * b + which] = v;
      } else {
        v = rd.in[t][2 * b + which];
      }
    }
    vals[e] = v;
  }
  __syncthreads();
  const uint32_t items = rd.num_terms * D * P;
  for (uint32_t it = threadIdx.x; it < items; it += blockDim.x) {
    const uint32_t pl = it % P, mx = it / P, x = mx % D, m = mx / D;
    Fr acc = Fr::zero();
    if (b0 + pl < size) {
      const int nf = rd.nfac[m];
      for (int k = 0; k <= nf; k++) {
        int t;
        if (k < nf) t = rd.fac[m][k];
        else if (rd.global_eq >= 0) t = rd.global_eq;
        else break;
        const Fr* pv = vals + ((uint32_t)g.slot_of[t] * P + pl) * 2;
        Fr v0 = pv[0], v1 = pv[1];
        Fr val = v1;
        if (x > 0) {
          Fr step = sub(v1, v0);
          for (uint32_t j = 0; j < x; j++) val = add(val, step);
        }
        acc = k == 0 ? val : mul(acc, val);
      }
    }
    red[it] = acc;
  }
  __syncthreads();
  const uint32_t groups = rd.num_terms * D;
  Fr gsum = Fr::zero();
  if (threadIdx.x < groups) {
    for (uint32_t pl = 0; pl < P; pl++) gsum = add(gsum, red[threadIdx.x * P + pl]);
    const uint32_t m = threadIdx.x / D;
    if (!rd.coeff_is_one[m]) gsum = mul(gsum, rd.coeff[m]);
  }
  __syncthreads();
// ... 294 lines not shown
  a.out_host = out_host;
  a.mbox = c.mbox();
  a.poll_ticks = (uint64_t)(knob(Knob::SC_TAIL_TIMEOUT_MS) * (double)c.wall_clock_khz);
  a.trace = nullptr;
  if (knob(Knob::SC_TAIL_TRACE) != 0) {
    a.trace = (uint64_t*)c.arena.alloc(32 * 8 * sizeof(uint64_t));
    LH_HIP(hipMemsetAsync(a.trace, 0, 32 * 8 * sizeof(uint64_t), c.stream));
    c.tail_trace = a.trace;
  }
  c.mbox_send(Fr::zero(), 0u);
  const size_t lds = ((size_t)a.red_off + tail_red_entries(rd, degree, a.cap)) * sizeof(Fr);
  c.opt_in_lds((const void*)sc_tail_kernel, (int)TAIL_LDS_BYTES + 2048);
  hipLaunchKernelGGL(sc_tail_kernel, dim3(G), dim3(G > 1 ? TAIL_THREADS_MULTI : TAIL_THREADS), lds, c.stream, a);
  LH_HIP(hipGetLastError());
}

void k_sc_tail_resync(Ctx& c) {
  LH_HIP(hipMemsetAsync(c.ticket + 32, 0, 4 * sizeof(TailChunk), c.stream));
  uint32_t v = 0;
  c.d2h(&v, c.ticket, sizeof(v));
  c.ticket_base = v;
}

bool k_sc_round_streams(const ScRound& rd, int degree, size_t size) {
  return !(rd.num_terms * (uint32_t)degree <= 256 && size * rd.num_terms <= ((size_t)1 << 16));
}

struct EqLevelsPack {
  const Fr* in;
  Fr* out[9];
};
__global__ __launch_bounds__(256) void eq_levels_kernel(EqLevelsPack pk, size_t n_in, int nlev) {
  const int lane = threadIdx.x & 63;
  const size_t waves = ((size_t)gridDim.x * blockDim.x) >> 6, tiles = (n_in + 511) / 512;
  for (size_t tile = ((size_t)blockIdx.x * blockDim.x + threadIdx.x) >> 6; tile < tiles; tile += waves) {
    Fr v[4];
#pragma unroll
    for (int r = 0; r < 4; r++) {
      const size_t i = tile * 512 + (size_t)r * 128 + 2 * (size_t)lane;
      v[r] = i + 1 < n_in ? add(pk.in[i], pk.in[i + 1]) : Fr::zero();
      if (nlev > 0 && (i >> 1) < (n_in >> 1)) pk.out[0][i >> 1] = v[r];
    }
#pragma unroll
    for (int k = 0; k < 6; k++) {
      const int lv = 1 + k;
#pragma unroll
      for (int r = 0; r < 4; r++) {
        Fr o;
#pragma unroll
        for (int q = 0; q < 8; q++) o.l[q] = __shfl_xor(v[r].l[q], 1 << k, 64);
        v[r] = add(v[r], o);
        if (lv < nlev && (lane & ((2 << k) - 1)) == 0) {
          const size_t idx = (tile * 256 + (size_t)r * 64 + (size_t)lane) >> (k + 1);
          if (idx < (n_in >> (lv + 1))) pk.out[lv][idx] = v[r];
        }
      }
    }
    if (lane == 0) {
      const Fr w0 = add(v[0], v[1]), w1 = add(v[2], v[3]);
      if (nlev > 7) {
        if (tile * 2 < (n_in >> 8)) pk.out[7][tile * 2] = w0;
        if (tile * 2 + 1 < (n_in >> 8)) pk.out[7][tile * 2 + 1] = w1;
      }
      if (nlev > 8 && tile < (n_in >> 9)) pk.out[8][tile] = add(w0, w1);
    }
  }
}
void k_eq_levels(Ctx& c, const Fr* in, size_t n_in, Fr* const* levels, size_t nlev) {
  size_t done = 0;
  while (done < nlev && n_in >= 2) {
    const size_t k = std::min<size_t>(9, nlev - done);
    EqLevelsPack pk;
    pk.in = in;
    for (size_t i = 0; i < 9; i++) pk.out[i] = i < k ? levels[done + i] : nullptr;
    const size_t waves = (n_in + 511) / 512;
    hipLaunchKernelGGL(eq_levels_kernel, dim3((unsigned)std::min<size_t>((waves + 3) / 4, 8192)), dim3(256), 0, c.stream, pk,
                       n_in, (int)k);
    in = levels[done + k - 1];
    n_in >>= k;
    done += k;
  }
}

static size_t sc_entry_grid(const Ctx& c, size_t entries) {
  constexpr size_t per_lane = 4;
  const size_t full = (entries + 255) / 256, cap = (size_t)c.num_cus * 8;
  size_t g = (entries + 256 * per_lane - 1) / (256 * per_lane);
  g = std::max(g, std::min(full, (size_t)c.num_cus * 2));
  return std::max<size_t>(1, std::min(std::min(g, full), cap));
}

template <int M, bool BIND>
__global__ __launch_bounds__(256) void sc_round_open_kernel(ScOpenRound rd, size_t size, Fr* __restrict__ partials, ScFinish fin) {
  __shared__ Fr lds[4];
  constexpr int NQ = 2 * M;
  Fr acc[M];
#pragma unroll
  for (int m = 0; m < M; m++) acc[m] = Fr::zero();
  const size_t items = 2 * size;
  const bool odd = threadIdx.x & 1;
  for (size_t i = (size_t)blockIdx.x * blockDim.x + threadIdx.x; i < items; i += (size_t)gridDim.x * blockDim.x) {
#pragma unroll
    for (int m = 0; m < M; m++) {
      const Fr v = load_entry<BIND>(rd.in[m], rd.out[m], i, rd.r, true);
      acc[m] = add(acc[m], mul(rd.eq_level[m][i >> 1], v));
    }
  }
#pragma unroll
  for (int m = 0; m < M; m++) {
    Fr q0, q1;
    reduce_by_parity(acc[m], odd, lds, q0, q1);
    if (threadIdx.x == 0) {
      fin_put(fin, partials, (size_t)blockIdx.x * NQ + 2 * m, q0);
      fin_put(fin, partials, (size_t)blockIdx.x * NQ + 2 * m + 1, q1);
    }
  }
  if (gridDim.x == 1) {
    if (threadIdx.x == 0) publish_round(fin, NQ);
    return;
  }
  finish_round<NQ>(fin, partials, lds);
}

template <int M>
static void launch_open(Ctx& c, const ScOpenRound& rd, bool bind, size_t size, unsigned g, Fr* partials, const ScFinish& fin) {
  if (bind)
    hipLaunchKernelGGL((sc_round_open_kernel<M, true>), dim3(g), dim3(256), 0, c.stream, rd, size, partials, fin);
  else
    hipLaunchKernelGGL((sc_round_open_kernel<M, false>), dim3(g), dim3(256), 0, c.stream, rd, size, partials, fin);
}

void k_sc_round_open(Ctx& c, const ScOpenRound& rd, bool bind, size_t size, Fr* out_host) {
  LH_REQUIRE(rd.num_terms >= 1 && rd.num_terms <= (uint32_t)SC_OPEN_MAX_TERMS && size >= 1, LH_ERR_ARG, "sc_round_open: bad shape");
  const uint32_t seq = c.next_seq();
  ArenaScope scope(c.arena);
  out_host = c.round_out(out_host);
  size_t g = sc_entry_grid(c, 2 * size);
  const int nq = 2 * (int)rd.num_terms;
  Fr* partials = g == 1 ? out_host : c.arena.alloc_n<Fr>(g * nq);
  const ScFinish fin = c.finish_for((uint32_t)g, out_host, seq, bind ? 64.0 * (double)size * rd.num_terms : 0.0);
  {
    ProfScope ps(c, bind ? "sc_round_open<bind>" : "sc_round_open<first>", ((bind ? 192.0 : 64.0) + 32.0) * (double)size * rd.num_terms,
                 (bind ? 4.0 : 2.0) * (double)size * rd.num_terms, (double)size);
    switch (rd.num_terms) {
      case 1: launch_open<1>(c, rd, bind, size, (unsigned)g, partials, fin); break;
      case 2: launch_open<2>(c, rd, bind, size, (unsigned)g, partials, fin); break;
      case 3: launch_open<3>(c, rd, bind, size, (unsigned)g, partials, fin); break;
      case 4: launch_open<4>(c, rd, bind, size, (unsigned)g, partials, fin); break;
      case 5: launch_open<5>(c, rd, bind, size, (unsigned)g, partials, fin); break;
      default: launch_open<6>(c, rd, bind, size, (unsigned)g, partials, fin); break;
    }
  }
  c.wait_round(seq);
}

template <int P, bool BIND, bool FOLD>
__global__ __launch_bounds__(256) void sc_round_rw_kernel(ScRwRound rd, size_t size, Fr* __restrict__ partials, ScFinish fin) {
  __shared__ Fr lds[4];
  Fr acc = Fr::zero();
  const size_t items = 2 * size;
  const bool odd = threadIdx.x & 1;
  for (size_t i = (size_t)blockIdx.x * blockDim.x + threadIdx.x; i < items; i += (size_t)gridDim.x * blockDim.x) {
    Fr av[P], bv[P];
#pragma unroll
    for (int p = 0; p < P; p++) {
      if (BIND && FOLD) {
        const Fr lf = mul(add(load_entry<true>(rd.l[p], rd.lo[p], i, rd.rchal, false), rd.k[p]), rd.cs[p]);
        const Fr rf = add(load_entry<true>(rd.r[p], rd.ro[p], i, rd.rchal, false), rd.k[p]);
        rd.lo[p][i] = lf, rd.ro[p][i] = rf;
        av[p] = at_lane_point(lf, odd), bv[p] = at_lane_point(rf, odd);
      } else {
        const Fr a = add(at_lane_point(load_entry<BIND>(rd.l[p], rd.lo[p], i, rd.rchal, true), odd), rd.k[p]);
        av[p] = mul(a, rd.cs[p]);
        bv[p] = add(at_lane_point(load_entry<BIND>(rd.r[p], rd.ro[p], i, rd.rchal, true), odd), rd.k[p]);
      }
    }
    acc = add(acc, mul(dot<FrParams, P>(av, bv), rd.eq_level[i >> 1]));
  }
  Fr q2, q1;
  reduce_by_parity(acc, odd, lds, q2, q1);
  if (threadIdx.x == 0) {
    fin_put(fin, partials, (size_t)blockIdx.x * 2, q1);
    fin_put(fin, partials, (size_t)blockIdx.x * 2 + 1, q2);
  }
  if (gridDim.x == 1) {
    if (threadIdx.x == 0) publish_round(fin, 2);
    return;
  }
  finish_round<2>(fin, partials, lds);
}

template <int P>
static void launch_rw(Ctx& c, const ScRwRound& rd, bool bind, bool fold, size_t size, unsigned g, Fr* partials, const ScFinish& fin) {
  if (bind && fold)
    hipLaunchKernelGGL((sc_round_rw_kernel<P, true, true>), dim3(g), dim3(256), 0, c.stream, rd, size, partials, fin);
  else if (bind)
    hipLaunchKernelGGL((sc_round_rw_kernel<P, true, false>), dim3(g), dim3(256), 0, c.stream, rd, size, partials, fin);
  else
    hipLaunchKernelGGL((sc_round_rw_kernel<P, false, false>), dim3(g), dim3(256), 0, c.stream, rd, size, partials, fin);
}

void k_sc_round_rw(Ctx& c, const ScRwRound& rd, bool bind, size_t size, Fr* out_host, bool fold) {
  LH_REQUIRE(!fold || bind, LH_ERR_ARG, "sc_round_rw: folding is part of a binding round");
  LH_REQUIRE(rd.num_pairs >= 1 && rd.num_pairs <= (uint32_t)SC_RW_MAX_PAIRS && size >= 1 && rd.eq_level, LH_ERR_ARG,
             "sc_round_rw: bad shape");
  const uint32_t seq = c.next_seq();
  ArenaScope scope(c.arena);
  out_host = c.round_out(out_host);
  size_t g = sc_entry_grid(c, 2 * size);
  Fr* partials = g == 1 ? out_host : c.arena.alloc_n<Fr>(g * 2);
  const ScFinish fin = c.finish_for((uint32_t)g, out_host, seq, bind ? 64.0 * (double)size * 2.0 * rd.num_pairs : 0.0);
  {
    const double P = (double)rd.num_pairs;
    ProfScope ps(c, bind ? "sc_round_rw<bind>" : "sc_round_rw<first>", ((bind ? 192.0 : 64.0) * 2.0 * P + 32.0) * (double)size,
                 ((bind ? 8.0 : 4.0) * P + 2.0) * (double)size, (double)size);
    switch (rd.num_pairs) {
      case 1: launch_rw<1>(c, rd, bind, fold, size, (unsigned)g, partials, fin); break;
      case 2: launch_rw<2>(c, rd, bind, fold, size, (unsigned)g, partials, fin); break;
      case 3: launch_rw<3>(c, rd, bind, fold, size, (unsigned)g, partials, fin); break;
      case 4: launch_rw<4>(c, rd, bind, fold, size, (unsigned)g, partials, fin); break;
      case 5: launch_rw<5>(c, rd, bind, fold, size, (unsigned)g, partials, fin); break;
      case 6: launch_rw<6>(c, rd, bind, fold, size, (unsigned)g, partials, fin); break;
      case 7: launch_rw<7>(c, rd, bind, fold, size, (unsigned)g, partials, fin); break;
      default: launch_rw<8>(c, rd, bind, fold, size, (unsigned)g, partials, fin); break;
    }
  }
  c.wait_round(seq);
}

bool k_sc_round(Ctx& c, const ScRound& rd, int degree, bool bind, size_t size, Fr* evals_host) {
  LH_REQUIRE(degree >= 1 && degree <= 6, LH_ERR_ARG, "sum-check degree must be in 1..6");
  LH_REQUIRE(size >= 1, LH_ERR_ARG, "sum-check round over an empty table");
  ScArgs a;
  a.rd = rd;
  bool seen[SC_MAX_TABLES] = {false};
  if (rd.global_eq >= 0) seen[rd.global_eq] = true;
  for (uint32_t m = 0; m < rd.num_terms; m++)
    for (int k = 0; k < rd.nfac[m]; k++) {
      int t = rd.fac[m][k];
      a.store[m][k] = seen[t] ? 0 : 1;
      seen[t] = true;
    }
  size_t tabs = 0;
  for (int t = 0; t < SC_MAX_TABLES; t++) tabs += seen[t] ? 1 : 0;
  double nfac = 0, ncoef = 0;
  for (uint32_t m = 0; m < rd.num_terms; m++) nfac += rd.nfac[m], ncoef += rd.coeff_is_one[m] ? 0 : 2;
  const double muls_pair = std::max(0.0, nfac - rd.num_terms) * degree + ncoef + (rd.global_eq >= 0 || rd.eq_level ? degree : 0) +
                           (bind ? 2.0 * (nfac + (rd.global_eq >= 0 ? 1 : 0)) : 0.0);
  const double bytes = (bind ? 192.0 : 64.0) * (double)size * (double)tabs + (rd.eq_level ? 32.0 * (double)size : 0.0);
  const uint32_t seq = c.next_seq();
  ArenaScope scope(c.arena);
  evals_host = c.round_out(evals_host);
  auto finish = [&](size_t grid, bool streams = false) {
    return c.finish_for((uint32_t)grid, evals_host, seq, streams && bind ? bytes / 3.0 : 0.0);
  };

  uint32_t P = (uint32_t)std::min<size_t>(size, 64);
  P = std::min<uint32_t>(P, LDS_VALS / (2 * (uint32_t)tabs));
  P = std::min<uint32_t>(P, LDS_ITEMS / (rd.num_terms * degree));
  const bool use_lds = P >= 1 && !rd.eq_level && !k_sc_round_streams(rd, degree, size);
  if (use_lds) {
    uint32_t want = (256 + rd.num_terms * degree - 1) / (rd.num_terms * degree);
    want = std::min<uint32_t>(want, std::max<uint32_t>(1, 256 / (2 * (uint32_t)tabs)));
    if (P > want && want >= 1) P = std::max<uint32_t>(want, 1);
    ScLdsArgs g;
    g.a = a;
    g.num_used = 0;
    for (int t = 0; t < SC_MAX_TABLES; t++)
      if (seen[t]) {
        g.slot_of[t] = (uint8_t)g.num_used;
        g.used[g.num_used++] = (uint8_t)t;
      }
    g.P = P;
    g.vals_entries = std::max<uint32_t>(g.num_used * P * 2, 8);
    size_t grid = (size + P - 1) / P;
    Fr* partials = grid == 1 ? evals_host : c.arena.alloc_n<Fr>(grid * degree);
    const ScFinish kflag = finish(grid);
    {
      char name[40];
      snprintf(name, sizeof name, "sc_round<%d,%s>/lds", degree, bind ? "bind" : "first");
      ProfScope ps(c, name, bytes, muls_pair * (double)size, (double)size);
      switch (degree) {
        case 1: launch_lds<1>(c, g, bind, size, (unsigned)grid, partials, kflag); break;
        case 2: launch_lds<2>(c, g, bind, size, (unsigned)grid, partials, kflag); break;
        case 3: launch_lds<3>(c, g, bind, size, (unsigned)grid, partials, kflag); break;
        case 4: launch_lds<4>(c, g, bind, size, (unsigned)grid, partials, kflag); break;
        case 5: launch_lds<5>(c, g, bind, size, (unsigned)grid, partials, kflag); break;
        default: launch_lds<6>(c, g, bind, size, (unsigned)grid, partials, kflag); break;
      }
    }
    c.wait_round(seq);
    return false;
  }

  const uint32_t tp = (rd.num_terms > 1 && size * rd.num_terms <= ((size_t)1 << 17)) ? rd.num_terms : 1u;
  if (degree == 2 && rd.eq_level && tp == 1) {
    size_t g2 = sc_entry_grid(c, 2 * size);
    Fr* partials = g2 == 1 ? evals_host : c.arena.alloc_n<Fr>(g2 * 2);
    const ScFinish kflag = finish(g2, true);
    if (rd.pp) {
      const double mp = (bind ? 2.0 * nfac : 0.0) + ncoef + 2.0 * 0.62 * rd.num_terms + 2.0;
      ProfScope ps(c, bind ? "sc_round_pp<bind>" : "sc_round_pp<first>", bytes, mp * (double)size, (double)size);
      if (bind) hipLaunchKernelGGL((sc_round_pp_kernel<true>), dim3((unsigned)g2), dim3(256), 0, c.stream, a, size, partials, kflag);
      else hipLaunchKernelGGL((sc_round_pp_kernel<false>), dim3((unsigned)g2), dim3(256), 0, c.stream, a, size, partials, kflag);
    } else {
      ProfScope ps(c, bind ? "sc_round<2,bind>" : "sc_round<2,first>", bytes, muls_pair * (double)size, (double)size);
      if (bind) hipLaunchKernelGGL((sc_round_e2_kernel<true>), dim3((unsigned)g2), dim3(256), 0, c.stream, a, size, partials, kflag);
      else hipLaunchKernelGGL((sc_round_e2_kernel<false>), dim3((unsigned)g2), dim3(256), 0, c.stream, a, size, partials, kflag);
    }
    c.wait_round(seq);
    return rd.pp == 2 && bind;
  }
  size_t g = (size * tp + 255) / 256;
  size_t cap = (size_t)c.num_cus * 4;
  if (g > cap) g = cap;
  Fr* partials = g == 1 ? evals_host : c.arena.alloc_n<Fr>(g * degree);
  const ScFinish kflag = finish(g, true);
  {
    char name[40];
    snprintf(name, sizeof name, "sc_round<%d,%s>%s", degree, bind ? "bind" : "first", tp > 1 ? "/tp" : "");
    ProfScope ps(c, name, bytes, muls_pair * (double)size, (double)size);
    switch (degree) {
      case 1: launch_round<1>(c, a, bind, size, tp, (unsigned)g, partials, kflag); break;
      case 2: launch_round<2>(c, a, bind, size, tp, (unsigned)g, partials, kflag); break;
      case 3: launch_round<3>(c, a, bind, size, tp, (unsigned)g, partials, kflag); break;
      case 4: launch_round<4>(c, a, bind, size, tp, (unsigned)g, partials, kflag); break;
      case 5: launch_round<5>(c, a, bind, size, tp, (unsigned)g, partials, kflag); break;
      default: launch_round<6>(c, a, bind, size, tp, (unsigned)g, partials, kflag); break;
    }
  }
  c.wait_round(seq);
  return false;
}

}
```

### halo2-lasso_amd/csrc/sumcheck.cpp

```cpp
#include <algorithm>
#include <functional>
#include <chrono>
#include <memory>
#include <thread>
#include "host.hpp"
#include "resident_host.hpp"

namespace lh {

std::vector<HFr> host_eq_xy(const std::vector<HFr>& y) {
  if (y.empty()) return {};
  std::vector<HFr> evals{HFr::one()};
  for (size_t i = y.size(); i-- > 0;) {
    std::vector<HFr> nxt(evals.size() * 2);
    for (size_t k = 0; k < evals.size(); k++) {
      nxt[2 * k + 1] = evals[k] * y[i];
      nxt[2 * k] = evals[k] - nxt[2 * k + 1];
    }
    evals.swap(nxt);
  }
  return evals;
}

HFr host_eq_xy_eval(const HFr* x, const HFr* y, size_t n) {
// ... 65 lines not shown
void comm_sum_points(Ctx& c, HG1* pts, size_t n) {
  const size_t R = (size_t)c.comm.size;
  std::vector<HG1> all(n * R);
  comm_all_gather_host(c, pts, all.data(), n * sizeof(HG1));
  std::vector<host::G1Xyzz> acc(n, host::G1Xyzz::identity());
  for (size_t i = 0; i < n; i++)
    for (size_t r = 0; r < R; r++) acc[i] = host::g1_add(acc[i], host::g1_from_affine(all[r * n + i]));
  host::g1_batch_to_affine(acc.data(), n, pts);
}

void comm_gather_tables(Ctx& c, const Fr* local_block, size_t count, size_t n_local, size_t block, Fr* const* out) {
  const size_t R = (size_t)c.comm.size;
  ArenaScope scope(c.arena);
  Fr* gathered = c.arena.alloc_n<Fr>(count * n_local * R);
  comm_all_gather_dev(c, local_block, gathered, count * n_local * sizeof(Fr));
  k_gather_interleave(c, gathered, count, n_local, R, block, out);
}

void comm_gather_concat(Ctx& c, const Fr* local, size_t n_local, Fr* out) {
  comm_all_gather_dev(c, local, out, n_local * sizeof(Fr));
}

static size_t log2_exact(size_t v) {
  size_t l = 0;
  while (((size_t)1 << l) < v) l++;
  return l;
}

void eq_xy_shard(Ctx& c, const Shard& sh, const HFr* y, size_t num_vars, size_t first, Fr* out_local) {
  std::vector<HFr> yl;
  HFr scale = HFr::one();
  for (size_t i = first; i < num_vars; i++) {
    if (i >= sh.j && i < sh.j + sh.rho) {
      bool bit = (sh.rank >> (i - sh.j)) & 1;
      scale *= bit ? y[i] : HFr::one() - y[i];
    } else {
      yl.push_back(y[i]);
    }
  }
  const size_t n_local = (size_t)1 << yl.size();
  k_eq_xy(c, (const Fr*)yl.data(), yl.size(), out_local);
  if (sh.rho) k_scale(c, out_local, dev(scale), n_local, out_local);
}

std::vector<HFr> evaluate_polys(Ctx& c, const Fr* const* d_polys, size_t count, size_t num_vars, const HFr* point, bool sharded) {
  if (!sharded) return evaluate_polys(c, d_polys, count, num_vars, point);
  std::vector<HFr> out(count);
  if (!count) return out;
  const Shard sh(c);
  ArenaScope scope(c.arena);
  const size_t n_local = (size_t)1 << (num_vars - sh.rho);
  Fr* eq = c.arena.alloc_n<Fr>(n_local);
  eq_xy_shard(c, sh, point, num_vars, 0, eq);
  k_inner_products(c, d_polys, count, eq, n_local, (Fr*)out.data());
  comm_sum_fr(c, out.data(), count);
  return out;
}

const Fr* eq_half_lookup(Ctx& c, const HFr* y, size_t num_vars, bool sharded) {
  if (num_vars < 2) return nullptr;
  const size_t bytes = (num_vars - 1) * sizeof(HFr);
  for (const Ctx::EqHalfEntry& e : c.eq_half_cache)
    if (e.sharded == sharded && e.key.size() == bytes && memcmp(e.key.data(), y + 1, bytes) == 0) return e.table;
  return nullptr;
}
const Fr* eq_half_get(Ctx& c, const HFr* y, size_t num_vars, bool sharded) {
  if (const Fr* t = eq_half_lookup(c, y, num_vars, sharded)) return t;
  LH_REQUIRE(num_vars >= 2, LH_ERR_ARG, "eq_half: needs two variables");
  Fr* t;
  if (sharded) {
    const Shard sh(c);
    t = c.arena.alloc_n<Fr>((size_t)1 << (num_vars - sh.rho - 1));
    eq_xy_shard(c, sh, y, num_vars, 1, t);
  } else {
    t = c.arena.alloc_n<Fr>((size_t)1 << (num_vars - 1));
    k_eq_xy(c, (const Fr*)(y + 1), num_vars - 1, t);
  }
  Ctx::EqHalfEntry e;
  e.key.assign((const uint8_t*)(y + 1), (const uint8_t*)(y + 1) + (num_vars - 1) * sizeof(HFr));
  e.table = t;
  e.sharded = sharded;
  c.eq_half_cache.push_back(std::move(e));
  return t;
}

SumCheckResult sum_check_loop(Ctx& c, int prover_kind, size_t num_vars, int degree, std::vector<const Fr*> cur,
                                     const std::vector<char>& used, size_t num_polys, const HFr& sum, Transcript& tr,
                                     bool sharded, const RoundFn& round_fn, const ScRound* tail_rd, EqFactoring* ef) {
  const size_t T = cur.size();
  bool ef_on = ef != nullptr;
  const size_t tail_cap = tail_rd ? k_sc_tail_capacity(c, *tail_rd, degree) : 0;
  const size_t rho = sharded ? log2_exact((size_t)c.comm.size) : 0, j = c.shard_bit;
  size_t len = (size_t)1 << (num_vars - rho);
  size_t x_round = 0;
  if (sharded) {
    x_round = j;
    for (size_t r = 1; r < j; r++)
      if ((T << (num_vars - r)) <= ((size_t)1 << c.opt.shard_exchange_log)) {
        x_round = r;
        break;
      }
  }
  std::vector<Fr*> bufA(T), bufB(T);
  auto alloc_bufs = [&](size_t l) {
    for (size_t i = 0; i < T; i++) {
      bufA[i] = c.arena.alloc_n<Fr>(std::max<size_t>(l >> 1, 1));
      bufB[i] = c.arena.alloc_n<Fr>(std::max<size_t>(l >> 2, 1));
    }
  };
  alloc_bufs(len);
  int flip = 0;
  Fr* evals_host = (Fr*)c.pin((16 + SC_MAX_TABLES) * sizeof(Fr));
  static const HFr inv2 = HFr::from_u64(2).inv();

  SumCheckResult res;
  HFr claim = sum;
  HFr r_prev = HFr::zero();
  bool sh = sharded;
  std::vector<HFr> pending;
  HFr pending_r;
  bool pending_coeffs = false;
  auto resolve_claim = [&] {
    if (pending.empty()) return;
    claim = pending_coeffs ? horner(pending, pending_r) : interpolate_evals(pending, pending_r);
    pending.clear();
  };
  auto message = [&](const Fr* sums) {
    resolve_claim();
    std::vector<HFr> ev(degree + 1);
    for (int x = 1; x <= degree; x++) ev[x] = hst(sums[x - 1]);
    ev[0] = claim - ev[1];
    HFr r;
    if (prover_kind == LH_SC_COEFFICIENTS) {
      std::vector<HFr> co(3);
      co[0] = ev[0];
      co[2] = (ev[2] - ev[1].dbl() + ev[0]) * inv2;
      co[1] = claim - (co[0].dbl() + co[2]);
      tr.write_field_elements(co);
      r = tr.squeeze_challenge();
      pending = std::move(co), pending_coeffs = true;
    } else {
      tr.write_field_elements(ev);
      r = tr.squeeze_challenge();
      pending = std::move(ev), pending_coeffs = false;
    }
    pending_r = r;
    res.challenges.push_back(r);
    return r;
  };
  bool factored_round = false;
  Fr *d_part = nullptr, *d_all = nullptr;
  bool tail_ok = true;
  bool resident_ok = true;
  for (size_t round = 0; round < num_vars; round++) {
    bool bind = round > 0;
    if (sh && round == x_round) {
      len >>= 1;
      std::vector<size_t> live;
      for (size_t i = 0; i < T; i++) {
        bool factored = false;
        if (ef_on)
          for (const EqFactoring::One& one : ef->eqs) factored = factored || one.table == i;
        if (!factored) live.push_back(i);
      }
      const size_t L = live.size();
      Fr* block = c.arena.alloc_n<Fr>(L * len);
      std::vector<const Fr*> src(L);
      std::vector<Fr*> dst(L), rep(L);
      for (size_t k = 0; k < L; k++) src[k] = cur[live[k]], dst[k] = block + k * len;
      k_fix_var_multi(c, src.data(), dst.data(), L, len << 1, dev(r_prev));
      const size_t full = len << rho;
      for (size_t k = 0; k < L; k++) rep[k] = c.arena.alloc_n<Fr>(full);
      comm_gather_tables(c, block, L, len, (size_t)1 << (j - round), rep.data());
      c.route.v[RouteStats::SHARD_EXCHANGES]++;
      for (size_t k = 0; k < L; k++) cur[live[k]] = rep[k];
      if (ef_on && tail_ok && ef->resident_tail && !ef->per_term && !ef->untrusted && full >= 4 && full <= ((size_t)GKR_CAP * GKR_CAP)) {
        EqFactoring::One& one = ef->eqs[0];
        Fr* lvl = c.arena.alloc_n<Fr>(full >> 1);
        k_eq_xy(c, (const Fr*)(one.y + round + 1), num_vars - round - 1, lvl);
        one.level[round] = lvl;
        resolve_claim();
        if (ef->resident_tail(cur, false, r_prev, full, round, claim, tr, res)) return res;
      }
      if (ef_on) {
        for (EqFactoring::One& one : ef->eqs) {
          Fr* tab = c.arena.alloc_n<Fr>(full);
          k_eq_xy(c, (const Fr*)(one.y + round), num_vars - round, tab);
          k_scale(c, tab, dev(one.S), full, tab);
          cur[one.table] = tab;
        }
        ef_on = false;
      }
      len = full;
      alloc_bufs(len);
      flip = 0;
      sh = false;
      bind = false;
    }
    if (ef_on && !sh && tail_ok && resident_ok && ef->resident_tail) {
      const size_t n0 = bind ? len >> 1 : len;
      if (n0 >= 2 && n0 <= ((size_t)GKR_CAP * GKR_CAP) && (round > 0 || ef->trusted_claim) && !ef->untrusted) {
        resolve_claim();
        if (ef->resident_tail(cur, bind, r_prev, n0, round, claim, tr, res)) return res;
        resident_ok = false;
      }
    }
    const bool tail_now = !sh && tail_ok && tail_cap && (bind ? len >> 1 : len) <= tail_cap;
    const bool keep_factored = tail_ok && resident_ok && ef_on && ef->resident_tail && !ef->per_term && !ef->untrusted &&
                               (sh || (bind ? len >> 1 : len) > ((size_t)GKR_CAP * GKR_CAP));
    if (ef_on && !keep_factored && (tail_now || !ef->streams(bind, bind ? len >> 2 : len >> 1))) {
      for (EqFactoring::One& one : ef->eqs) {
        Fr* tab = c.arena.alloc_n<Fr>(len);
        if (round >= 2) {
          LH_REQUIRE(bind, LH_ERR_ARG, "sum-check: internal round mismatch");
          k_scale(c, one.level[round - 2], dev(one.S_prev), len, tab);
        } else if (sharded) {
          eq_xy_shard(c, Shard(c), one.y, num_vars, 0, tab);
        } else {
          k_eq_xy(c, (const Fr*)one.y, num_vars, tab);
        }
        cur[one.table] = tab;
      }
      ef_on = false;
    }
    if (tail_now) {
      const size_t n0 = bind ? len >> 1 : len, rounds = num_vars - round;
      LH_REQUIRE(((size_t)1 << rounds) == n0 && num_polys <= T, LH_ERR_ARG, "sum-check: internal size mismatch");
      ScRound rd = *tail_rd;
      for (size_t i = 0; i < T; i++) rd.in[i] = cur[i], rd.out[i] = nullptr;
      rd.r = dev(r_prev);
      const uint32_t seq0 = c.flag_seq + 1;
      c.flag_seq += (uint32_t)rounds + 1;
      const bool tail_debug = knob(Knob::SC_DEBUG) != 0;
      const auto t_tail = std::chrono::steady_clock::now();
      ProfScope ps(c, "sc_tail", 0, 0, (double)n0);
      struct Guard {
        Ctx& c;
        bool done = false;
        ~Guard() {
          if (done) return;
          c.mbox_abort();
          (void)hipStreamSynchronize(c.stream);
          try {
            k_sc_tail_resync(c);
          } catch (...) {
          }
        }
      } guard{c};
      TailChunk* chunks = (TailChunk*)evals_host;
      memset((void*)chunks, 0, 3 * SC_TAIL_MAX_DEGREE * sizeof(TailChunk));
      k_sc_tail_launch(c, rd, degree, n0, bind, num_polys, seq0, chunks, evals_host + 16);
      c.route.v[RouteStats::TAILS]++;
      double host_us = 0;
      size_t absorbed = 0;
      bool gave_up = false;
      Fr sums[SC_TAIL_MAX_DEGREE];
      auto wait = [&](uint32_t seq, bool msg) {
        try {
          if (msg) c.wait_chunks(chunks, 3 * (size_t)degree, seq, sums);
          else c.wait_flag(seq);
          return true;
        } catch (const Error& e) {
          if (e.code != LH_ERR_DEVICE || hipStreamQuery(c.stream) != hipSuccess) throw;
          return false;
        }
      };
      for (size_t i = 0; i < rounds && !gave_up; i++) {
        if (!wait(seq0 + (uint32_t)i, true)) {
          gave_up = true;
          break;
        }
        const auto t_h = std::chrono::steady_clock::now();
        const HFr r = message(sums);
        c.mbox_send(dev(r), seq0 + (uint32_t)i);
        absorbed = i + 1;
        c.route.v[RouteStats::TAIL_ROUNDS]++;
        if (tail_debug) host_us += std::chrono::duration<double, std::micro>(std::chrono::steady_clock::now() - t_h).count();
      }
      if (!gave_up && !wait(seq0 + (uint32_t)rounds, false)) gave_up = true;
      guard.done = true;
      if (!gave_up && c.tail_trace) {
        std::vector<uint64_t> st(rounds * 8);
        c.d2h(st.data(), c.tail_trace, st.size() * sizeof(uint64_t));
        c.tail_trace = nullptr;
        const double tick_us = 1e3 / (double)c.wall_clock_khz;
        fprintf(stderr, "[sc_tail trace] T %zu degree %d n0 %zu\n", T, degree, n0);
        for (size_t i = 0; i < rounds; i++) {
          const uint64_t* s8 = &st[i * 8];
          auto rel = [&](int k) { return s8[k] ? (double)(int64_t)(s8[k] - s8[0]) * tick_us : -1.0; };
          fprintf(stderr, "  round %2zu: eval %.2f ticket %.2f last-sees %.2f sent %.2f challenge %.2f | next round starts %.2f\n", i,
                  rel(1), rel(2), rel(3), rel(4), rel(5),
                  i + 1 < rounds && st[(i + 1) * 8] ? (double)(int64_t)(st[(i + 1) * 8] - s8[0]) * tick_us : -1.0);
        }
      }
      if (!gave_up) {
        if (tail_debug)
          fprintf(stderr, "[sc_tail] T %zu terms %u degree %d n0 %zu rounds %zu: %.1f us (host side %.1f us)\n", T,
                  tail_rd->num_terms, degree, n0, rounds,
// ... 240 lines not shown
  if (ef_enabled && nvl >= 3 && (!sharded || j >= 2) && (streams2 || tail_shape)) {
    if (rd.global_eq >= 0 && prover_kind == LH_SC_EVALUATIONS && degree >= 2 && (!sharded || sum_is_exact)) {
      bool ok = true;
      for (uint32_t m = 0; m < rd.num_terms && ok; m++)
        for (int k = 0; k < rd.nfac[m]; k++) ok = ok && rd.fac[m][k] != rd.global_eq;
      const HFr* y = ys + (size_t)expr.global_eq * num_vars;
      std::vector<HFr> d(num_vars);
      for (size_t i = 0; i < num_vars && ok; i++) {
        d[i] = HFr::one() - y[i];
        ok = !d[i].is_zero();
      }
      if (ok) {
        std::vector<HFr> pre(num_vars + 1);
        pre[0] = HFr::one();
        for (size_t i = 0; i < num_vars; i++) pre[i + 1] = pre[i] * d[i];
        HFr inv = pre[num_vars].inv();
        ef.inv_1my.resize(num_vars);
        for (size_t i = num_vars; i-- > 0;) {
          ef.inv_1my[i] = inv * pre[i];
          inv = inv * d[i];
        }
        ef.per_term = false;
        ef.trusted_claim = sum_is_exact;
        ef.c = sum;
        EqFactoring::One one;
        one.table = (size_t)rd.global_eq, one.y = y, one.S = one.S_prev = HFr::one();
        ef.eqs.push_back(one);
        use_ef = true;
      }
    } else if (rd.global_eq < 0 && prover_kind == LH_SC_COEFFICIENTS && rd.num_terms <= (uint32_t)SC_OPEN_MAX_TERMS &&
               T == 2 * (size_t)rd.num_terms) {
      bool ok = true;
      std::vector<char> seen(T, 0);
      for (uint32_t m = 0; m < rd.num_terms && ok; m++) {
        ok = rd.nfac[m] == 2 && rd.coeff_is_one[m];
        if (!ok) break;
        size_t a = rd.fac[m][0], b = rd.fac[m][1];
        if (a < num_polys) std::swap(a, b);
        ok = a >= num_polys && b < num_polys && !seen[a] && !seen[b];
        if (!ok) break;
        seen[a] = seen[b] = 1;
        EqFactoring::One one;
        one.table = a, one.y = ys + (a - num_polys) * num_vars, one.S = one.S_prev = HFr::one();
        ef.eqs.push_back(one);
        term_poly.push_back(b);
      }
      ef.per_term = true;
      use_ef = ok;
    }
  }
  ScU32 u32s = u32;
  Fr u32_r0;
  bool u32_bound = false;
  if (u32.col) {
    const bool u32_off = knob(Knob::SC_U32) == 0;
    u32_rounds = !u32_off && use_ef && !ef.per_term && !sharded && !rw && num_polys == 1 && rd.num_terms == 1 && rd.nfac[0] == 1 &&
                 rd.fac[0][0] == 0 && rd.coeff_is_one[0] && degree == 2 && sum_is_exact && streams2 && num_vars >= 6 &&
                 k_sc_round_streams(rd, degree, len0 >> 3) &&
                 (len0 >> 2) > std::max<size_t>(k_sc_tail_capacity(c, rd, degree), (size_t)GKR_CAP * GKR_CAP);
    if (!u32_rounds) k_fr_from_u32(c, u32.col, len0, const_cast<Fr*>(d_polys[0]));
  }
  std::vector<Fr> u32t_sums;
  Fr u32t_r0;
  if (!u32t.polys.empty()) {
    const bool u32t_off = knob(Knob::OPEN_U32_ROUNDS) == 0;
    LH_REQUIRE(u32t.polys.size() == num_polys, LH_ERR_ARG, "sum-check: the column hint does not match the polys");
    bool ok = !u32t_off && use_ef && ef.per_term && !sharded && degree == 2 && streams2 && num_vars >= 22 &&
              k_sc_round_streams(rd, degree, len0 >> 3) &&
              (len0 >> 2) > std::max<size_t>(k_sc_tail_capacity(c, rd, degree), (size_t)GKR_CAP * GKR_CAP);
    for (const ScU32Terms::Poly& pl : u32t.polys) {
      ok = ok && !pl.col.empty() && pl.col.size() <= 24;
      for (size_t ln : pl.len) ok = ok && ln % 4 == 0;
    }
    u32t_rounds = ok;
    if (!ok)
      for (size_t b = 0; b < num_polys; b++) {
        const ScU32Terms::Poly& pl = u32t.polys[b];
        k_lincomb_mixed(c, nullptr, nullptr, 0, pl.col.data(), pl.len.data(), pl.w.data(), pl.col.size(), len0, const_cast<Fr*>(d_polys[b]));
      }
  }
  const bool pp_shape = use_ef && !ef.per_term && pp_terms;
  std::vector<HFr> pp_folded;
  bool rw_folded = false;
  if (use_ef) {
    const Shard shg(c);
    const size_t half = (size_t)1 << (nvl - 1);
    for (EqFactoring::One& one : ef.eqs) {
      const Fr* shared = eq_half_lookup(c, one.y, num_vars, sharded);
      Fr* buf = c.arena.alloc_n<Fr>(shared ? half : 2 * half);
      one.level.resize(num_vars);
      size_t off = 0;
      for (size_t jl = 0; jl < nvl; jl++) {
        if (jl == 0 && shared) {
          one.level[0] = const_cast<Fr*>(shared);
          continue;
        }
        one.level[jl] = buf + off;
        off += half >> jl;
      }
      if (!shared) {
        if (sharded) eq_xy_shard(c, shg, one.y, num_vars, 1, buf);
        else k_eq_xy(c, (const Fr*)(one.y + 1), num_vars - 1, buf);
      }
      std::vector<Fr*> lower;
      for (size_t jl = 1; jl < nvl; jl++) lower.push_back((Fr*)one.level[jl]);
      k_eq_levels(c, one.level[0], half, lower.data(), lower.size());
    }
    ef.streams = [&](bool, size_t size) { return k_sc_round_streams(rd, degree, size); };
    ef.round = [&](const Fr* const* in, Fr* const* out, const Fr& r, bool bind, size_t size, size_t round, int points,
                   Fr* out_host) {
      if (!ef.per_term && rw && rw_folded) {
        LH_REQUIRE(points == 2, LH_ERR_ARG, "sum-check: tree-pair rounds asked for an extra point after the fold");
        ScRound g;
        memset(&g, 0, sizeof(g));
        g.num_tables = 2 * rw->num_pairs, g.num_terms = rw->num_pairs;
        for (size_t i = 0; i < 2 * (size_t)rw->num_pairs; i++) g.in[i] = in[i], g.out[i] = out[i];
        for (uint32_t m = 0; m < rw->num_pairs; m++) {
          g.coeff[m] = dev(HFr::one()), g.coeff_is_one[m] = 1;
          g.nfac[m] = 2, g.fac[m][0] = (uint8_t)(2 * m), g.fac[m][1] = (uint8_t)(2 * m + 1);
        }
        g.r = r;
        g.global_eq = -1;
        g.eq_level = ef.eqs[0].level[round];
        g.pp = 1;
        k_sc_round(c, g, points, bind, size, out_host);
        ef.add_const = rw->const_total;
      } else if (!ef.per_term && rw && points == 2) {
        ScRwRound g;
        memset(&g, 0, sizeof(g));
        g.num_pairs = rw->num_pairs;
        for (uint32_t i = 0; i < rw->num_pairs; i++) {
          g.l[i] = in[2 * i], g.r[i] = in[2 * i + 1];
          g.lo[i] = out[2 * i], g.ro[i] = out[2 * i + 1];
          g.cs[i] = dev(rw->cs[i]), g.k[i] = dev(rw->k[i]);
        }
        g.eq_level = ef.eqs[0].level[round];
        g.rchal = r;
        const bool fold = bind && c.opt.sc_pp_fold == 1;
        k_sc_round_rw(c, g, bind, size, out_host, fold);
        if (fold) {
          rw_folded = true;
          c.route.v[RouteStats::PP_FOLDS]++;
          const uint32_t P = rw->num_pairs;
          rd.num_terms = P + 1;
          for (uint32_t m = 0; m < P; m++) {
            rd.coeff[m] = dev(HFr::one()), rd.coeff_is_one[m] = 1;
            rd.nfac[m] = 2, rd.fac[m][0] = (uint8_t)(2 * m), rd.fac[m][1] = (uint8_t)(2 * m + 1);
          }
          rd.coeff[P] = dev(rw->const_total), rd.coeff_is_one[P] = 0, rd.nfac[P] = 0;
        }
        c.route.v[RouteStats::RW_ROUNDS]++;
        ef.add_const = rw->const_total;
      } else if (!ef.per_term && u32_rounds && round <= 2) {
        LH_REQUIRE(points == 1 && bind == (round >= 1), LH_ERR_ARG, "sum-check: the 32-bit rounds met another shape");
        if (round == 0) {
          if (!u32s.have_sums) {
            Fr s4[4];
            k_inner_products_small_quads(c, u32.col, ef.eqs[0].level[0], size >> 1, s4);
            u32s.odd = s4[1], u32s.s2 = s4[2], u32s.s3 = s4[3], u32s.have_sums = true;
          }
          out_host[0] = u32s.odd;
        } else if (round == 1) {
          u32_r0 = r;
          const HFr r0 = hst(r);
          out_host[0] = dev((HFr::one() - r0) * hst(u32s.s2) + r0 * hst(u32s.s3));
        } else {
          k_sc_round_u32_bind2(c, u32.col, ef.eqs[0].level[2], u32_r0, r, size, out[0], out_host);
          u32_bound = true;
        }
      } else if (!ef.per_term) {
        ScRound g = rd;
        for (size_t i = 0; i < T; i++) g.in[i] = in[i], g.out[i] = out[i];
        g.r = r;
        g.global_eq = -1;
        g.eq_level = ef.eqs[0].level[round];
        g.pp = pp_shape && points == 2 ? 1 : 0;
        if (g.pp && bind && pp_folded.empty() && c.opt.sc_pp_fold == 1) g.pp = 2;
        if (k_sc_round(c, g, points, bind, size, out_host)) {
          pp_folded.resize(rd.num_terms);
          for (uint32_t m = 0; m < rd.num_terms; m++) {
            memcpy(&pp_folded[m], &rd.coeff[m], 32);
            rd.coeff[m] = dev(HFr::one());
            rd.coeff_is_one[m] = 1;
          }
          c.route.v[RouteStats::PP_FOLDS]++;
        }
      } else if (u32t_rounds && round <= 2) {
        LH_REQUIRE(bind == (round >= 1), LH_ERR_ARG, "sum-check: the column rounds met another shape");
        const uint32_t M = rd.num_terms;
        if (round == 0) {
          ArenaScope scope(c.arena);
          size_t total = 0;
          for (uint32_t m = 0; m < M; m++) total += u32t.polys[term_poly[m]].col.size();
          Fr* d_s = c.arena.alloc_n<Fr>(4 * total);
          size_t off = 0;
          for (uint32_t m = 0; m < M; m++) {
            const ScU32Terms::Poly& pl = u32t.polys[term_poly[m]];
            k_inner_products_quads(c, pl.col.data(), pl.len.data(), pl.col.size(), ef.eqs[m].level[1], size >> 1, d_s + 4 * off);
            off += pl.col.size();
          }
          std::vector<Fr> hs(4 * total);
          c.d2h(hs.data(), d_s, hs.size() * sizeof(Fr));
          u32t_sums.assign(4 * (size_t)M, dev(HFr::zero()));
          off = 0;
          for (uint32_t m = 0; m < M; m++) {
            const ScU32Terms::Poly& pl = u32t.polys[term_poly[m]];
            HFr t4[4] = {HFr::zero(), HFr::zero(), HFr::zero(), HFr::zero()};
            for (size_t k = 0; k < pl.col.size(); k++)
              for (int t = 0; t < 4; t++) t4[t] += hst(pl.w[k]) * hst(hs[4 * (off + k) + t]);
            off += pl.col.size();
            for (int t = 0; t < 4; t++) u32t_sums[4 * m + t] = dev(t4[t]);
            const HFr y1 = ef.eqs[m].y[1], n1 = HFr::one() - y1;
            out_host[2 * m] = dev(n1 * t4[0] + y1 * t4[2]);
            out_host[2 * m + 1] = dev(n1 * t4[1] + y1 * t4[3]);
          }
        } else if (round == 1) {
          u32t_r0 = r;
          const HFr r0 = hst(r), n0 = HFr::one() - r0;
          for (uint32_t m = 0; m < M; m++) {
            const Fr* t4 = &u32t_sums[4 * m];
            out_host[2 * m] = dev(n0 * hst(t4[0]) + r0 * hst(t4[1]));
            out_host[2 * m + 1] = dev(n0 * hst(t4[2]) + r0 * hst(t4[3]));
          }
        } else {
          Fr* two = (Fr*)c.pin(65536) + 1024;
          for (uint32_t m = 0; m < M; m++) {
            const ScU32Terms::Poly& pl = u32t.polys[term_poly[m]];
            k_lincomb_bind2(c, pl.col.data(), pl.len.data(), pl.w.data(), pl.col.size(), u32t_r0, r, ef.eqs[m].level[2], size,
                            out[term_poly[m]], two);
            out_host[2 * m] = two[0], out_host[2 * m + 1] = two[1];
          }
          u32t_bound = true;
        }
      } else {
        ScOpenRound g;
        g.num_terms = rd.num_terms;
        g.r = r;
        for (uint32_t m = 0; m < rd.num_terms; m++) {
          g.in[m] = in[term_poly[m]], g.out[m] = out[term_poly[m]];
          g.eq_level[m] = ef.eqs[m].level[round];
        }
        k_sc_round_open(c, g, bind, size, out_host);
      }
    };
  }
  if (use_ef && !ef.per_term && c.opt.gkr_resident && c.opt.sc_tail && (pp_shape || rw) && num_polys == 2 * (size_t)(rw ? rw->num_pairs : rd.num_terms) &&
      (rw ? rw->num_pairs : rd.num_terms) <= (uint32_t)GKR_MAX_TREES) {
    ef.resident_tail = [&](const std::vector<const Fr*>& cur_t, bool bind, const HFr& r_prev, size_t n0, size_t round,
                           const HFr& claim_now, Transcript& trr, SumCheckResult& res) {
      const size_t Bt = rw ? rw->num_pairs : rd.num_terms;
      GkrLayerDev L;
      memset(&L, 0, sizeof(L));
      L.B = (uint32_t)Bt;
      L.flags = GKR_F_SPLIT | GKR_F_NOMSG | GKR_F_EQ | (bind ? GKR_F_BIND : 0) | (rw && !rw_folded ? GKR_F_KOFF : 0);
      std::vector<size_t> li(Bt), ri(Bt);
      std::vector<HFr> co(Bt), ko(Bt, HFr::zero());
      for (size_t m = 0; m < Bt; m++) {
        li[m] = rw ? 2 * m : rd.fac[m][0], ri[m] = rw ? 2 * m + 1 : rd.fac[m][1];
        if (rw && rw_folded) co[m] = HFr::one();
        else if (rw) co[m] = rw->cs[m], ko[m] = rw->k[m];
        else memcpy(&co[m], &rd.coeff[m], 32);
        if (co[m].is_zero()) return false;
        L.lv[m] = cur_t[li[m]], L.rv[m] = cur_t[ri[m]];
        L.coef[m] = dev(co[m]), L.koff[m] = dev(ko[m]);
      }
      EqFactoring::One& e = ef.eqs[0];
      L.eq_level = e.level[round];
      L.r_prev = dev(r_prev);
      std::vector<HFr> x, finals;
      if (!resident_tail_run(c, L, n0, e.y + round, ef.inv_1my.data() + round, e.S, ef.c, claim_now, rw ? rw->const_total : HFr::zero(),
                             trr, x, finals))
        return false;
      res.challenges.insert(res.challenges.end(), x.begin(), x.end());
      std::vector<HFr> pre(Bt + 1);
      pre[0] = HFr::one();
      for (size_t m = 0; m < Bt; m++) pre[m + 1] = pre[m] * co[m];
      HFr inv = pre[Bt].inv();
      res.evals.assign(num_polys, HFr::zero());
      for (size_t m = Bt; m-- > 0;) {
        res.evals[li[m]] = finals[2 * m] * (inv * pre[m]) - ko[m];
        res.evals[ri[m]] = finals[2 * m + 1] - ko[m];
        inv = inv * co[m];
      }
      return true;
    };
  }
  for (size_t jy = 0; jy < num_ys; jy++) {
    bool factored = false;
    if (use_ef)
      for (const EqFactoring::One& one : ef.eqs) factored = factored || one.table == num_polys + jy;
    if (factored) continue;
    Fr* eq = c.arena.alloc_n<Fr>(len0);
    if (sharded) eq_xy_shard(c, Shard(c), ys + jy * num_vars, num_vars, 0, eq);
    else k_eq_xy(c, (const Fr*)(ys + jy * num_vars), num_vars, eq);
    cur[num_polys + jy] = eq;
  }
  SumCheckResult res = sum_check_loop(c, prover_kind, num_vars, degree, cur, used, num_polys, sum, tr, sharded, round_fn, &rd,
                                      use_ef ? &ef : nullptr);
  LH_REQUIRE(!u32_rounds || u32_bound, LH_ERR_DEVICE, "sum-check: the 32-bit column was never bound");
  LH_REQUIRE(!u32t_rounds || u32t_bound, LH_ERR_DEVICE, "sum-check: the 32-bit columns were never bound");
  res.u32_terms_built = !u32t.polys.empty() && !u32t_rounds;
  if (rw_folded) {
    const size_t K = rw->num_pairs;
    std::vector<HFr> pre(K + 1);
    pre[0] = HFr::one();
    for (size_t m = 0; m < K; m++) pre[m + 1] = pre[m] * rw->cs[m];
    HFr inv = pre[K].inv();
    for (size_t m = K; m-- > 0;) {
      res.evals[2 * m] = res.evals[2 * m] * (inv * pre[m]) - rw->k[m];
      res.evals[2 * m + 1] = res.evals[2 * m + 1] - rw->k[m];
      inv = inv * rw->cs[m];
    }
  }
  if (!pp_folded.empty()) {
    const size_t K = pp_folded.size();
    std::vector<HFr> pre(K + 1);
    pre[0] = HFr::one();
    for (size_t m = 0; m < K; m++) pre[m + 1] = pre[m] * pp_folded[m];
    HFr inv = pre[K].inv();
    for (size_t m = K; m-- > 0;) {
      res.evals[rd.fac[m][0]] = res.evals[rd.fac[m][0]] * (inv * pre[m]);
      inv = inv * pp_folded[m];
    }
  }
  return res;
}

}
```

### include/lasso_hip.h

```cpp
#ifndef LASSO_HIP_H
#define LASSO_HIP_H

#include <stddef.h>
#include <stdint.h>

#ifdef __cplusplus
extern "C" {
#endif

typedef struct { uint64_t l[4]; } lh_fr;
typedef struct { uint64_t x[4], y[4]; } lh_g1;

typedef int lh_status;
#define LH_OK 0
#define LH_ERR_INVALID_SUMCHECK (-1)
#define LH_ERR_INVALID_PCS_PARAM (-2)
#define LH_ERR_INVALID_PCS_OPEN (-3)
#define LH_ERR_INVALID_SNARK (-4)
#define LH_ERR_SERIALIZATION (-5)
#define LH_ERR_TRANSCRIPT (-6)
#define LH_ERR_DEVICE (-7)
#define LH_ERR_ARG (-8)

typedef struct lh_ctx lh_ctx;
// ... 71 lines not shown
#define LH_EX_NEGATED 6
#define LH_EX_SUM 7
#define LH_EX_PRODUCT 8
#define LH_EX_SCALED 9
typedef struct lh_expr_node { uint32_t op; int32_t a, b; uint32_t reserved; lh_fr scalar; } lh_expr_node;
typedef struct lh_expr { const lh_expr_node* nodes; size_t num_nodes; } lh_expr;
lh_status lh_sumcheck_prove_expr(lh_ctx*, size_t num_vars, const lh_expr* expr, const lh_fr* const* d_polys,
                                 size_t num_polys, const lh_fr* challenges, size_t num_challenges,
                                 const lh_fr* ys, size_t num_ys, const lh_fr* sum, lh_transcript* t,
                                 lh_fr* out_challenges, lh_fr* out_evals);

lh_status lh_gkr_fractional_prove(lh_ctx*, size_t num_batching, size_t num_vars,
                                  const lh_fr* const* claimed_p_0s, const lh_fr* const* claimed_q_0s,
                                  const lh_fr* const* d_ps, const lh_fr* const* d_qs,
                                  lh_transcript* t, lh_fr* out_p_xs, lh_fr* out_q_xs, lh_fr* out_x);
lh_status lh_grand_product_prove(lh_ctx*, size_t num_trees, const lh_fr* const* d_leaves,
                                 const size_t* num_vars, lh_transcript* t, lh_fr* out_roots,
                                 lh_fr* out_claims, lh_fr* out_points);

lh_status lh_msm(lh_ctx*, const lh_fr* d_scalars, const lh_g1* d_bases, size_t n, lh_g1* out);
lh_status lh_msm_u32(lh_ctx*, const uint32_t* d_scalars, const lh_g1* d_bases, size_t n, lh_g1* out);

typedef struct lh_srs lh_srs;
lh_status lh_mkzg_setup(lh_ctx*, const lh_fr* ss, size_t num_vars, lh_srs** out);
lh_status lh_srs_upload(lh_ctx*, const lh_g1* eqs_flat, size_t num_vars, lh_srs** out);
lh_status lh_srs_download(lh_ctx*, const lh_srs*, lh_g1* eqs_flat);
size_t lh_srs_num_vars(const lh_srs*);
void lh_srs_free(lh_ctx*, lh_srs*);
lh_status lh_mkzg_commit(lh_ctx*, const lh_srs*, const lh_fr* d_poly, size_t num_vars, lh_g1* out);
lh_status lh_mkzg_batch_commit(lh_ctx*, const lh_srs*, const lh_fr* const* d_polys, size_t num_polys,
                               size_t num_vars, lh_g1* out_comms);
lh_status lh_mkzg_open(lh_ctx*, const lh_srs*, const lh_fr* d_poly, size_t num_vars,
                       const lh_fr* point, lh_transcript* t, lh_fr* out_eval);
typedef struct lh_evaluation { uint32_t poly, point; lh_fr value; } lh_evaluation;
lh_status lh_mkzg_batch_open(lh_ctx*, const lh_srs*, size_t num_vars,
                             const lh_fr* const* d_polys, size_t num_polys,
                             const lh_fr* points, size_t num_points,
                             const lh_evaluation* evals, size_t num_evals, lh_transcript* t);

#define LH_SUBTABLE_IDENTITY 0
#define LH_SUBTABLE_AND 1
#define LH_SUBTABLE_XOR 2
#define LH_LASSO_MAX_CHUNKS 8
#define LH_LASSO_MAX_MEMORIES 16
#define LH_LASSO_MAX_TERMS 16
typedef struct lh_lasso_table {
  uint32_t num_chunks;
  uint32_t chunk_bits;
  uint32_t num_memories;
  uint32_t memory_chunk[LH_LASSO_MAX_MEMORIES];
  uint32_t memory_subtable[LH_LASSO_MAX_MEMORIES];
  uint32_t num_terms;
  lh_fr g_coeff[LH_LASSO_MAX_TERMS];
  uint8_t g_num_factors[LH_LASSO_MAX_TERMS];
  uint8_t g_factor[LH_LASSO_MAX_TERMS][LH_SC_MAX_FACTORS];
} lh_lasso_table;
lh_status lh_lasso_prove(lh_ctx*, const lh_srs*, const lh_lasso_table*, size_t num_vars,
                         const uint32_t* const* d_dims, lh_transcript* t);

#define LH_LASSO_NUM_PHASES 9
lh_status lh_lasso_last_timing(lh_ctx*, double* out_ms);

lh_status lh_ctx_set_option(lh_ctx*, const char* name, int64_t value);
lh_status lh_ctx_get_option(lh_ctx*, const char* name, int64_t* out);
#define LH_LASSO_ROUTE_WORDS 24
typedef struct lh_lasso_route {
  uint32_t open_small_depth;
  uint32_t open_small_passes;
  uint32_t eq_factored_rounds;
  uint32_t standard_rounds;
  uint32_t rw_leaf_rounds;
  uint32_t resident_tails;
  uint32_t resident_rounds;
  uint32_t packed_ts_pairs;
  uint32_t derived_commitments;
  uint32_t sorted_dim_reuse;
  uint32_t sharded_rounds;
  uint32_t shard_exchanges;
  uint32_t window_table_jobs;
  uint32_t open_precommit;
  uint32_t resident_layers;
  uint32_t pp_folds;
  uint32_t msm_half_batches;
  uint32_t reserved[7];
} lh_lasso_route;
lh_status lh_lasso_last_route(lh_ctx*, lh_lasso_route* out);

typedef struct lh_comm {
  int rank, size;
  void* user;
  int (*all_gather)(void* user, const void* send, void* recv, size_t bytes_per_rank);
  int (*all_gather_device)(void* user, const void* d_send, void* d_recv, size_t bytes_per_rank, void* hip_stream);
} lh_comm;
lh_status lh_ctx_set_comm(lh_ctx*, const lh_comm* comm, size_t shard_bit);
#define LH_RCCL_UNIQUE_ID_BYTES 128
lh_status lh_rccl_unique_id(uint8_t out[LH_RCCL_UNIQUE_ID_BYTES]);
lh_status lh_ctx_set_comm_rccl(lh_ctx*, int rank, int size, const uint8_t unique_id[LH_RCCL_UNIQUE_ID_BYTES],
                               size_t shard_bit);
lh_status lh_ctx_set_comm_loopback(lh_ctx*, int rank, int size, size_t shard_bit);
lh_status lh_ctx_comm_stats(lh_ctx*, uint64_t out[2]);
lh_status lh_ctx_comm_phase_stats(lh_ctx*, uint64_t out[16], int reset);
lh_status lh_ctx_memory_stats(lh_ctx*, uint64_t out[4]);
lh_status lh_ctx_host_cpus(lh_ctx*, char* bus_id, size_t bus_id_cap, char* cpulist, size_t cpulist_cap);
lh_status lh_lasso_prove_sharded(lh_ctx*, const lh_srs*, const lh_lasso_table*, size_t num_vars,
                                 const uint32_t* const* d_dims_local, lh_transcript* t);

typedef struct lh_hp_lookup {
  const lh_expr* inputs;
  const lh_expr* tables;
  size_t width;
} lh_hp_lookup;
#define LH_HP_LASSO_MAX_COMMITMENTS 63
typedef struct lh_hp_lasso_lookup {
  lh_lasso_table table;
  size_t output_poly;
  size_t chunk_polys[LH_LASSO_MAX_CHUNKS];
} lh_hp_lasso_lookup;
typedef struct lh_hp_param {
  size_t num_vars;
  size_t num_instance_polys;
  const size_t* num_instances;
  size_t num_preprocess_polys;
  const void* const* d_preprocess_polys;
  size_t num_witness_polys;
  size_t num_challenges;
  size_t num_lookups;
  const lh_hp_lookup* lookups;
  size_t num_permutation_polys;
  const size_t* permutation_poly_index;
  const void* const* d_permutation_polys;
  size_t num_permutation_z_polys;
  lh_expr expression;
  size_t num_lasso_lookups;
  const lh_hp_lasso_lookup* lasso_lookups;
} lh_hp_param;
lh_status lh_hyperplonk_prove(lh_ctx*, const lh_srs*, const lh_hp_param*, const lh_fr* const* instances,
                              const lh_fr* const* d_witness_polys, lh_transcript* t);

lh_status lh_shard_extract(lh_ctx*, const void* d_global, size_t n_local, size_t shard_bit, size_t rho, size_t rank,
                           size_t elem_bytes, void* d_local);
lh_status lh_hyperplonk_prove_sharded(lh_ctx*, const lh_srs*, const lh_hp_param*, const lh_fr* const* instances,
                                      const lh_fr* const* d_witness_polys_local, lh_transcript* t);

typedef struct lh_hp_circuit {
  void* user;
  int (*synthesize)(void* user, size_t round, const lh_fr* challenges, size_t num_challenges,
                    const void** d_out_polys, size_t num_out);
} lh_hp_circuit;
lh_status lh_hyperplonk_prove_phases(lh_ctx*, const lh_srs*, const lh_hp_param*, size_t num_phases,
                                     const size_t* num_witness_polys, const size_t* num_challenges,
                                     const lh_fr* const* instances, const lh_hp_circuit* circuit, lh_transcript* t);

typedef struct lh_g2 { uint64_t x_c0[4], x_c1[4], y_c0[4], y_c1[4]; } lh_g2;
typedef struct lh_mkzg_vp lh_mkzg_vp;
lh_status lh_mkzg_vp_setup(const lh_fr* ss, size_t num_vars, lh_mkzg_vp** out);
lh_status lh_mkzg_vp_new(const lh_g1* g1, const lh_g2* g2, const lh_g2* ss, size_t num_vars, lh_mkzg_vp** out);
lh_status lh_mkzg_vp_export(const lh_mkzg_vp*, lh_g1* g1, lh_g2* g2, lh_g2* ss);
size_t lh_mkzg_vp_num_vars(const lh_mkzg_vp*);
void lh_mkzg_vp_free(lh_mkzg_vp*);
lh_status lh_pairing_check(const lh_g1* ps, const lh_g2* qs, size_t n, int* out_is_identity);
lh_status lh_mkzg_verify(const lh_mkzg_vp*, const lh_g1* comm, const lh_fr* point, size_t num_vars,
                         const lh_fr* eval, lh_transcript* t);
lh_status lh_mkzg_batch_verify(const lh_mkzg_vp*, size_t num_vars, const lh_g1* comms, size_t num_comms,
                               const lh_fr* points, size_t num_points, const lh_evaluation* evals,
                               size_t num_evals, lh_transcript* t);
lh_status lh_sumcheck_verify(int prover_kind, size_t num_vars, size_t degree, const lh_fr* sum,
                             lh_transcript* t, lh_fr* out_eval, lh_fr* out_x);
// ... 208 lines not shown
```

Measured before the change: 55.31 ms.

## Split eq tables into hi/lo factors for large sum-check rounds

Large eq-factored sum-check rounds no longer materialise a full eq level table per round. Each level is represented as the product of a small shared high-variable table and a per-round low table, and the low factor is applied once per thread at the end of the grid-stride loop. This cuts the memory traffic and allocation needed to build and stream the eq tables. In exchange the grid size is constrained to multiples of the low-table span, and full levels are rebuilt lazily when the resident tail or scale path needs them. A new cap option limits the size of resident GKR layers.

Result: no change. 54.98 ms (median of 4 runs) (-0.6%).

```diff
diff --git a/bindings/rust/src/sys.rs b/bindings/rust/src/sys.rs
--- a/bindings/rust/src/sys.rs
+++ b/bindings/rust/src/sys.rs
@@ -177,7 +177,8 @@
     pub resident_layers: u32,
     pub pp_folds: u32,
     pub msm_half_batches: u32,
-    pub reserved: [u32; 7],
+    pub eq_split_rounds: u32,
+    pub reserved: [u32; 6],
 }
 
 extern "C" {
diff --git a/halo2-lasso_amd/__init__.py b/halo2-lasso_amd/__init__.py
--- a/halo2-lasso_amd/__init__.py
+++ b/halo2-lasso_amd/__init__.py
@@ -1466,7 +1466,8 @@
 
 ROUTE_FIELDS = ["open_small_depth", "open_small_passes", "eq_factored_rounds", "standard_rounds", "rw_leaf_rounds",
                 "resident_tails", "resident_rounds", "packed_ts_pairs", "derived_commitments", "sorted_dim_reuse",
-                "sharded_rounds", "shard_exchanges", "window_table_jobs", "open_precommit", "resident_layers", "pp_folds", "msm_half_batches"]
+                "sharded_rounds", "shard_exchanges", "window_table_jobs", "open_precommit", "resident_layers", "pp_folds", "msm_half_batches",
+                "eq_split_rounds"]
 
 
 def lasso_last_route(ctx):
diff --git a/halo2-lasso_amd/csrc/dev.cpp b/halo2-lasso_amd/csrc/dev.cpp
--- a/halo2-lasso_amd/csrc/dev.cpp
+++ b/halo2-lasso_amd/csrc/dev.cpp
@@ -82,7 +82,8 @@
     {"shard_exchange_log", &Options::shard_exchange_log, 0, 40},   {"msm_window_tables", &Options::msm_window_tables, 0, 40},
     {"open_precommit", &Options::open_precommit, 0, 64},           {"gkr_resident", &Options::gkr_resident, 0, 1},
     {"sc_pp_fold", &Options::sc_pp_fold, 0, 2},                    {"msm_half_batches", &Options::msm_half_batches, 0, 1},
-    {"comm_round", &Options::comm_round, 0, 2},
+    {"comm_round", &Options::comm_round, 0, 2},                    {"sc_eq_split_log", &Options::sc_eq_split_log, 0, 40},
+    {"gkr_resident_max_log", &Options::gkr_resident_max_log, 1, 14},
 };
 
 int64_t* Options::find(const char* name) {
diff --git a/halo2-lasso_amd/csrc/dev.hpp b/halo2-lasso_amd/csrc/dev.hpp
--- a/halo2-lasso_amd/csrc/dev.hpp
+++ b/halo2-lasso_amd/csrc/dev.hpp
@@ -107,6 +107,8 @@
   int64_t sc_pp_fold = 1;
   int64_t msm_half_batches = 1;
   int64_t gkr_resident = 1;
+  int64_t sc_eq_split_log = 13;
+  int64_t gkr_resident_max_log = 14;
   int64_t comm_round = 0;
   Options();
   int64_t* find(const char* name);
@@ -128,7 +130,7 @@
 struct RouteStats {
   uint32_t v[LH_LASSO_ROUTE_WORDS] = {0};
   enum { OPEN_DEPTH, OPEN_PASSES, EF_ROUNDS, STD_ROUNDS, RW_ROUNDS, TAILS, TAIL_ROUNDS, PACKED_TS, DERIVED, SORTED_REUSE,
-         SHARDED_ROUNDS, SHARD_EXCHANGES, WIN_TABLE_JOBS, OPEN_PRECOMMIT, RESIDENT_LAYERS, PP_FOLDS, MSM_HALF_BATCHES };
+         SHARDED_ROUNDS, SHARD_EXCHANGES, WIN_TABLE_JOBS, OPEN_PRECOMMIT, RESIDENT_LAYERS, PP_FOLDS, MSM_HALF_BATCHES, EQ_SPLIT_ROUNDS };
 };
 
 class HostWorker {
@@ -421,11 +423,17 @@
   uint8_t fac[LH_SC_MAX_TERMS][LH_SC_MAX_FACTORS];
   Fr r;
   const Fr* eq_level;
+  const Fr* eq_lo;
+  const Fr* eq_hi;
+  uint32_t eq_shift;
   uint8_t pp;
 };
 bool k_sc_round(Ctx&, const ScRound& rd, int degree, bool bind, size_t size, Fr* evals_host);
 bool k_sc_round_streams(const ScRound& rd, int degree, size_t size);
 void k_eq_levels(Ctx&, const Fr* in, size_t n_in, Fr* const* levels, size_t nlev);
+constexpr int EQ_SPLIT_MAX_VARS = 40;
+size_t k_eq_split_entries(size_t nv, size_t split_log, size_t* h);
+void k_eq_split(Ctx&, const Fr* y, size_t nv, size_t split_log, Fr* buf, const Fr** hi, const Fr** lo, const Fr** plain);
 constexpr int SC_OPEN_MAX_TERMS = 6;
 struct ScOpenRound {
   const Fr* in[SC_OPEN_MAX_TERMS];
@@ -444,6 +452,8 @@
   Fr* ro[SC_RW_MAX_PAIRS];
   Fr cs[SC_RW_MAX_PAIRS], k[SC_RW_MAX_PAIRS];
   const Fr* eq_level;
+  const Fr *eq_lo, *eq_hi;
+  uint32_t eq_shift;
   Fr rchal;
   uint32_t num_pairs;
 };
diff --git a/halo2-lasso_amd/csrc/gkr.cpp b/halo2-lasso_amd/csrc/gkr.cpp
--- a/halo2-lasso_amd/csrc/gkr.cpp
+++ b/halo2-lasso_amd/csrc/gkr.cpp
@@ -213,7 +213,7 @@
       GkrLayerDev L;
       memset(&L, 0, sizeof(L));
       uint32_t nb = 0;
-      bool ok = !sh.sharded(h + 1) && k_gkr_resident_geometry((uint32_t)h, &L.g, &L.s_log);
+      bool ok = !sh.sharded(h + 1) && h <= (size_t)c.opt.gkr_resident_max_log && k_gkr_resident_geometry((uint32_t)h, &L.g, &L.s_log);
       bool any_leaf = false, all_leaf = true;
       for (size_t b = 0; b < B && ok; b++) {
         if (num_vars[b] <= h) continue;
diff --git a/halo2-lasso_amd/csrc/host.hpp b/halo2-lasso_amd/csrc/host.hpp
--- a/halo2-lasso_amd/csrc/host.hpp
+++ b/halo2-lasso_amd/csrc/host.hpp
@@ -154,6 +154,9 @@
     size_t table;
     const HFr* y;
     std::vector<const Fr*> level;
+    const Fr* hi = nullptr;
+    std::vector<const Fr*> lo;
+    std::vector<uint32_t> shift;
     HFr S, S_prev;
     std::vector<HFr> q;
   };
diff --git a/halo2-lasso_amd/csrc/kernels_poly.hip b/halo2-lasso_amd/csrc/kernels_poly.hip
--- a/halo2-lasso_amd/csrc/kernels_poly.hip
+++ b/halo2-lasso_amd/csrc/kernels_poly.hip
@@ -262,6 +262,59 @@
     cur = dst;
     done += cnt[k];
   }
+}
+
+struct EqSplitArgs {
+  Fr y[EQ_SPLIT_MAX_VARS];
+  uint32_t end[2 * EQ_SPLIT_MAX_VARS + 2];
+  uint8_t first[2 * EQ_SPLIT_MAX_VARS + 2], nvars[2 * EQ_SPLIT_MAX_VARS + 2];
+  uint32_t num_tables;
+  Fr* buf;
+};
+__global__ __launch_bounds__(256) void eq_split_kernel(EqSplitArgs a) {
+  const uint32_t i = blockIdx.x * blockDim.x + threadIdx.x;
+  if (i >= a.end[a.num_tables - 1]) return;
+  uint32_t t = 0;
+  while (i >= a.end[t]) t++;
+  const uint32_t b = i - (t ? a.end[t - 1] : 0u);
+  Fr e = Fr::one();
+  for (uint32_t k = 0; k < a.nvars[t]; k++) {
+    const Fr yk = a.y[a.first[t] + k];
+    e = mul(e, (b >> k) & 1 ? yk : sub(Fr::one(), yk));
+  }
+  a.buf[i] = e;
+}
+static size_t eq_split_h(size_t nv, size_t split_log) { return std::max<size_t>(2, std::min(split_log, (nv + 1) / 2)); }
+size_t k_eq_split_entries(size_t nv, size_t split_log, size_t* h_out) {
+  const size_t h = eq_split_h(nv, split_log);
+  if (h_out) *h_out = h;
+  size_t total = (size_t)1 << h;
+  for (size_t j = 0; j <= nv; j++) total += (size_t)1 << (nv - j > split_log ? nv - j - h : nv - j);
+  return total;
+}
+void k_eq_split(Ctx& c, const Fr* y, size_t nv, size_t split_log, Fr* buf, const Fr** hi, const Fr** lo, const Fr** plain) {
+  LH_REQUIRE(nv <= (size_t)EQ_SPLIT_MAX_VARS && split_log >= 2 && nv > split_log, LH_ERR_ARG, "eq_split: bad shape");
+  const size_t h = eq_split_h(nv, split_log);
+  EqSplitArgs a;
+  memset(&a, 0, sizeof(a));
+  for (size_t k = 0; k < nv; k++) a.y[k] = y[k];
+  a.buf = buf;
+  uint32_t off = 0, t = 0;
+  auto table = [&](size_t first, size_t nvars) {
+    const Fr* p = buf + off;
+    off += (uint32_t)1 << nvars;
+    a.first[t] = (uint8_t)first, a.nvars[t] = (uint8_t)nvars, a.end[t++] = off;
+    return p;
+  };
+  *hi = table(nv - h, h);
+  for (size_t j = 0; j <= nv; j++) {
+    const bool split = nv - j > split_log;
+    lo[j] = split ? table(j, nv - j - h) : nullptr;
+    plain[j] = split ? nullptr : table(j, nv - j);
+  }
+  a.num_tables = t;
+  ProfScope ps(c, "eq_split", 32.0 * off, (double)h * off, (double)off);
+  hipLaunchKernelGGL(eq_split_kernel, dim3((off + 255) / 256), dim3(256), 0, c.stream, a);
 }
 
 template <class T>
diff --git a/halo2-lasso_amd/csrc/kernels_sumcheck.hip b/halo2-lasso_amd/csrc/kernels_sumcheck.hip
--- a/halo2-lasso_amd/csrc/kernels_sumcheck.hip
+++ b/halo2-lasso_amd/csrc/kernels_sumcheck.hip
@@ -99,8 +99,8 @@
 #pragma unroll
       for (int x = 0; x < D; x++) s[x] = add(s[x], pm[x]);
     }
-    if (rd.eq_level) {
-      const Fr e = rd.eq_level[b];
+    if (rd.eq_level || rd.eq_hi) {
+      const Fr e = rd.eq_level ? rd.eq_level[b] : mul(rd.eq_lo[b & (((size_t)1 << rd.eq_shift) - 1)], rd.eq_hi[b >> rd.eq_shift]);
 #pragma unroll
       for (int x = 0; x < D; x++) s[x] = mul(s[x], e);
     } else if (rd.global_eq >= 0) {
@@ -155,6 +155,18 @@
   odd_sum = block_reduce_sum(odd ? acc : Fr::zero(), lds);
 }
 
+struct EqFactor {
+  const Fr* __restrict__ tab;
+  const Fr* lo;
+  uint32_t shift;
+  __device__ __forceinline__ EqFactor(const Fr* level, const Fr* lo_, const Fr* hi, uint32_t shift_)
+      : tab(level ? level : hi), lo(level ? nullptr : lo_), shift(level ? 0u : shift_) {}
+  __device__ __forceinline__ Fr at(size_t pair) const { return tab[pair >> shift]; }
+  __device__ __forceinline__ Fr finish(const Fr& acc, size_t first_pair) const {
+    return lo ? mul(acc, lo[first_pair & (((size_t)1 << shift) - 1)]) : acc;
+  }
+};
+
 template <bool BIND>
 __global__ __launch_bounds__(256) void sc_round_e2_kernel(ScArgs a, size_t size, Fr* __restrict__ partials, ScFinish fin) {
   __shared__ Fr lds[4];
@@ -162,6 +174,7 @@
   Fr acc = Fr::zero();
   const size_t items = 2 * size;
   const bool odd = threadIdx.x & 1;
+  const EqFactor eq(rd.eq_level, rd.eq_lo, rd.eq_hi, rd.eq_shift);
   for (size_t i = (size_t)blockIdx.x * blockDim.x + threadIdx.x; i < items; i += (size_t)gridDim.x * blockDim.x) {
     Fr s = Fr::zero();
     for (uint32_t m = 0; m < rd.num_terms; m++) {
@@ -174,8 +187,9 @@
       }
       s = add(s, pm);
     }
-    acc = add(acc, mul(s, rd.eq_level[i >> 1]));
-  }
+    acc = add(acc, mul(s, eq.at(i >> 1)));
+  }
+  acc = eq.finish(acc, ((size_t)blockIdx.x * blockDim.x + threadIdx.x) >> 1);
   Fr q2, q1;
   reduce_by_parity(acc, odd, lds, q2, q1);
   if (threadIdx.x == 0) {
@@ -199,6 +213,7 @@
   const bool fold = BIND && rd.pp == 2;
   const uint32_t K = rd.num_terms;
   const Fr rch = rd.r;
+  const EqFactor eq(rd.eq_level, rd.eq_lo, rd.eq_hi, rd.eq_shift);
   for (size_t i = (size_t)blockIdx.x * blockDim.x + threadIdx.x; i < items; i += (size_t)gridDim.x * blockDim.x) {
     Fr s = Fr::zero();
     for (uint32_t m0 = 0; m0 < K; m0 += 4) {
@@ -240,8 +255,9 @@
       }
       s = add(s, dot<FrParams, 4>(av, bv));
     }
-    acc = add(acc, mul(s, rd.eq_level[i >> 1]));
-  }
+    acc = add(acc, mul(s, eq.at(i >> 1)));
+  }
+  acc = eq.finish(acc, ((size_t)blockIdx.x * blockDim.x + threadIdx.x) >> 1);
   Fr q2, q1;
   reduce_by_parity(acc, odd, lds, q2, q1);
   if (threadIdx.x == 0) {
@@ -702,12 +718,18 @@
   }
 }
 
-static size_t sc_entry_grid(const Ctx& c, size_t entries) {
+static size_t sc_entry_grid(const Ctx& c, size_t entries, uint32_t lo_shift = 0) {
   constexpr size_t per_lane = 4;
   const size_t full = (entries + 255) / 256, cap = (size_t)c.num_cus * 8;
   size_t g = (entries + 256 * per_lane - 1) / (256 * per_lane);
   g = std::max(g, std::min(full, (size_t)c.num_cus * 2));
-  return std::max<size_t>(1, std::min(std::min(g, full), cap));
+  g = std::max<size_t>(1, std::min(std::min(g, full), cap));
+  if (lo_shift > 7) {
+    const size_t unit = (size_t)1 << (lo_shift - 7);
+    g = std::max(g / unit * unit, unit);
+    LH_REQUIRE(unit <= full, LH_ERR_ARG, "sum-check: a split eq factor over too few pairs");
+  }
+  return g;
 }
 
 template <int M, bool BIND>
@@ -780,6 +802,7 @@
   Fr acc = Fr::zero();
   const size_t items = 2 * size;
   const bool odd = threadIdx.x & 1;
+  const EqFactor eq(rd.eq_level, rd.eq_lo, rd.eq_hi, rd.eq_shift);
   for (size_t i = (size_t)blockIdx.x * blockDim.x + threadIdx.x; i < items; i += (size_t)gridDim.x * blockDim.x) {
     Fr av[P], bv[P];
 #pragma unroll
@@ -795,8 +818,9 @@
         bv[p] = add(at_lane_point(load_entry<BIND>(rd.r[p], rd.ro[p], i, rd.rchal, true), odd), rd.k[p]);
       }
     }
-    acc = add(acc, mul(dot<FrParams, P>(av, bv), rd.eq_level[i >> 1]));
-  }
+    acc = add(acc, mul(dot<FrParams, P>(av, bv), eq.at(i >> 1)));
+  }
+  acc = eq.finish(acc, ((size_t)blockIdx.x * blockDim.x + threadIdx.x) >> 1);
   Fr q2, q1;
   reduce_by_parity(acc, odd, lds, q2, q1);
   if (threadIdx.x == 0) {
@@ -822,17 +846,18 @@
 
 void k_sc_round_rw(Ctx& c, const ScRwRound& rd, bool bind, size_t size, Fr* out_host, bool fold) {
   LH_REQUIRE(!fold || bind, LH_ERR_ARG, "sc_round_rw: folding is part of a binding round");
-  LH_REQUIRE(rd.num_pairs >= 1 && rd.num_pairs <= (uint32_t)SC_RW_MAX_PAIRS && size >= 1 && rd.eq_level, LH_ERR_ARG,
-             "sc_round_rw: bad shape");
+  LH_REQUIRE(rd.num_pairs >= 1 && rd.num_pairs <= (uint32_t)SC_RW_MAX_PAIRS && size >= 1 &&
+                 (rd.eq_level || (rd.eq_lo && rd.eq_hi && ((size_t)4 << rd.eq_shift) <= size)),
+             LH_ERR_ARG, "sc_round_rw: bad shape");
   const uint32_t seq = c.next_seq();
   ArenaScope scope(c.arena);
   out_host = c.round_out(out_host);
-  size_t g = sc_entry_grid(c, 2 * size);
+  size_t g = sc_entry_grid(c, 2 * size, rd.eq_level ? 0 : rd.eq_shift);
   Fr* partials = g == 1 ? out_host : c.arena.alloc_n<Fr>(g * 2);
   const ScFinish fin = c.finish_for((uint32_t)g, out_host, seq, bind ? 64.0 * (double)size * 2.0 * rd.num_pairs : 0.0);
   {
     const double P = (double)rd.num_pairs;
-    ProfScope ps(c, bind ? "sc_round_rw<bind>" : "sc_round_rw<first>", ((bind ? 192.0 : 64.0) * 2.0 * P + 32.0) * (double)size,
+    ProfScope ps(c, bind ? "sc_round_rw<bind>" : "sc_round_rw<first>", ((bind ? 192.0 : 64.0) * 2.0 * P + (rd.eq_level ? 32.0 : 0.0)) * (double)size,
                  ((bind ? 8.0 : 4.0) * P + 2.0) * (double)size, (double)size);
     switch (rd.num_pairs) {
       case 1: launch_rw<1>(c, rd, bind, fold, size, (unsigned)g, partials, fin); break;
@@ -853,6 +878,8 @@
   LH_REQUIRE(size >= 1, LH_ERR_ARG, "sum-check round over an empty table");
   ScArgs a;
   a.rd = rd;
+  const bool eq_factored = rd.eq_level || rd.eq_hi;
+  LH_REQUIRE(rd.eq_level || !rd.eq_hi || (rd.eq_lo && ((size_t)4 << rd.eq_shift) <= size), LH_ERR_ARG, "sum-check: bad split eq factor");
   bool seen[SC_MAX_TABLES] = {false};
   if (rd.global_eq >= 0) seen[rd.global_eq] = true;
   for (uint32_t m = 0; m < rd.num_terms; m++)
@@ -865,7 +892,7 @@
   for (int t = 0; t < SC_MAX_TABLES; t++) tabs += seen[t] ? 1 : 0;
   double nfac = 0, ncoef = 0;
   for (uint32_t m = 0; m < rd.num_terms; m++) nfac += rd.nfac[m], ncoef += rd.coeff_is_one[m] ? 0 : 2;
-  const double muls_pair = std::max(0.0, nfac - rd.num_terms) * degree + ncoef + (rd.global_eq >= 0 || rd.eq_level ? degree : 0) +
+  const double muls_pair = std::max(0.0, nfac - rd.num_terms) * degree + ncoef + (rd.global_eq >= 0 || eq_factored ? degree : 0) +
                            (bind ? 2.0 * (nfac + (rd.global_eq >= 0 ? 1 : 0)) : 0.0);
   const double bytes = (bind ? 192.0 : 64.0) * (double)size * (double)tabs + (rd.eq_level ? 32.0 * (double)size : 0.0);
   const uint32_t seq = c.next_seq();
@@ -878,7 +905,7 @@
   uint32_t P = (uint32_t)std::min<size_t>(size, 64);
   P = std::min<uint32_t>(P, LDS_VALS / (2 * (uint32_t)tabs));
   P = std::min<uint32_t>(P, LDS_ITEMS / (rd.num_terms * degree));
-  const bool use_lds = P >= 1 && !rd.eq_level && !k_sc_round_streams(rd, degree, size);
+  const bool use_lds = P >= 1 && !eq_factored && !k_sc_round_streams(rd, degree, size);
   if (use_lds) {
     uint32_t want = (256 + rd.num_terms * degree - 1) / (rd.num_terms * degree);
     want = std::min<uint32_t>(want, std::max<uint32_t>(1, 256 / (2 * (uint32_t)tabs)));
@@ -914,8 +941,8 @@
   }
 
   const uint32_t tp = (rd.num_terms > 1 && size * rd.num_terms <= ((size_t)1 << 17)) ? rd.num_terms : 1u;
-  if (degree == 2 && rd.eq_level && tp == 1) {
-    size_t g2 = sc_entry_grid(c, 2 * size);
+  if (degree == 2 && eq_factored && tp == 1) {
+    size_t g2 = sc_entry_grid(c, 2 * size, rd.eq_level ? 0 : rd.eq_shift);
     Fr* partials = g2 == 1 ? evals_host : c.arena.alloc_n<Fr>(g2 * 2);
     const ScFinish kflag = finish(g2, true);
     if (rd.pp) {
diff --git a/halo2-lasso_amd/csrc/sumcheck.cpp b/halo2-lasso_amd/csrc/sumcheck.cpp
--- a/halo2-lasso_amd/csrc/sumcheck.cpp
+++ b/halo2-lasso_amd/csrc/sumcheck.cpp
@@ -171,6 +171,16 @@
   e.sharded = sharded;
   c.eq_half_cache.push_back(std::move(e));
   return t;
+}
+
+static size_t resident_cap(const Ctx& c) { return std::min((size_t)GKR_CAP * GKR_CAP, (size_t)1 << c.opt.gkr_resident_max_log); }
+static const Fr* eq_level_full(Ctx& c, EqFactoring::One& one, size_t num_vars, size_t round) {
+  if (!one.level[round]) {
+    Fr* t = c.arena.alloc_n<Fr>((size_t)1 << (num_vars - 1 - round));
+    k_eq_xy(c, (const Fr*)(one.y + round + 1), num_vars - 1 - round, t);
+    one.level[round] = t;
+  }
+  return one.level[round];
 }
 
 SumCheckResult sum_check_loop(Ctx& c, int prover_kind, size_t num_vars, int degree, std::vector<const Fr*> cur,
@@ -263,7 +273,7 @@
       comm_gather_tables(c, block, L, len, (size_t)1 << (j - round), rep.data());
       c.route.v[RouteStats::SHARD_EXCHANGES]++;
       for (size_t k = 0; k < L; k++) cur[live[k]] = rep[k];
-      if (ef_on && tail_ok && ef->resident_tail && !ef->per_term && !ef->untrusted && full >= 4 && full <= ((size_t)GKR_CAP * GKR_CAP)) {
+      if (ef_on && tail_ok && ef->resident_tail && !ef->per_term && !ef->untrusted && full >= 4 && full <= resident_cap(c)) {
         EqFactoring::One& one = ef->eqs[0];
         Fr* lvl = c.arena.alloc_n<Fr>(full >> 1);
         k_eq_xy(c, (const Fr*)(one.y + round + 1), num_vars - round - 1, lvl);
@@ -288,21 +298,21 @@
     }
     if (ef_on && !sh && tail_ok && resident_ok && ef->resident_tail) {
       const size_t n0 = bind ? len >> 1 : len;
-      if (n0 >= 2 && n0 <= ((size_t)GKR_CAP * GKR_CAP) && (round > 0 || ef->trusted_claim) && !ef->untrusted) {
+      if (n0 >= 2 && n0 <= resident_cap(c) && (round > 0 || ef->trusted_claim) && !ef->untrusted) {
         resolve_claim();
         if (ef->resident_tail(cur, bind, r_prev, n0, round, claim, tr, res)) return res;
         resident_ok = false;
       }
     }
-    const bool tail_now = !sh && tail_ok && tail_cap && (bind ? len >> 1 : len) <= tail_cap;
     const bool keep_factored = tail_ok && resident_ok && ef_on && ef->resident_tail && !ef->per_term && !ef->untrusted &&
-                               (sh || (bind ? len >> 1 : len) > ((size_t)GKR_CAP * GKR_CAP));
+                               (sh || (bind ? len >> 1 : len) > resident_cap(c));
+    const bool tail_now = !keep_factored && !sh && tail_ok && tail_cap && (bind ? len >> 1 : len) <= tail_cap;
     if (ef_on && !keep_factored && (tail_now || !ef->streams(bind, bind ? len >> 2 : len >> 1))) {
       for (EqFactoring::One& one : ef->eqs) {
         Fr* tab = c.arena.alloc_n<Fr>(len);
         if (round >= 2) {
           LH_REQUIRE(bind, LH_ERR_ARG, "sum-check: internal round mismatch");
-          k_scale(c, one.level[round - 2], dev(one.S_prev), len, tab);
+          k_scale(c, eq_level_full(c, one, num_vars, round - 2), dev(one.S_prev), len, tab);
         } else if (sharded) {
           eq_xy_shard(c, Shard(c), one.y, num_vars, 0, tab);
         } else {
@@ -709,10 +719,30 @@
   const bool pp_shape = use_ef && !ef.per_term && pp_terms;
   std::vector<HFr> pp_folded;
   bool rw_folded = false;
+  auto set_eq = [&](auto& g, size_t round) {
+    const EqFactoring::One& e = ef.eqs[0];
+    g.eq_level = e.level[round];
+    if (g.eq_level) return;
+    g.eq_lo = e.lo[round], g.eq_hi = e.hi, g.eq_shift = e.shift[round];
+    c.route.v[RouteStats::EQ_SPLIT_ROUNDS]++;
+  };
   if (use_ef) {
     const Shard shg(c);
     const size_t half = (size_t)1 << (nvl - 1);
+    const size_t split_log = std::max<size_t>((size_t)c.opt.sc_eq_split_log, 2);
+    const bool split = c.opt.sc_eq_split_log != 0 && !ef.per_term && !sharded && !c.shard_active && !u32_rounds && nvl - 1 > split_log &&
+                       nvl - 1 <= (size_t)EQ_SPLIT_MAX_VARS && !eq_half_lookup(c, ef.eqs[0].y, num_vars, false);
+    if (split) {
+      EqFactoring::One& one = ef.eqs[0];
+      const size_t nv = nvl - 1;
+      size_t h;
+      Fr* buf = c.arena.alloc_n<Fr>(k_eq_split_entries(nv, split_log, &h));
+      one.level.resize(nv + 1), one.lo.resize(nv + 1), one.shift.resize(nv + 1);
+      k_eq_split(c, (const Fr*)(one.y + 1), nv, split_log, buf, &one.hi, one.lo.data(), one.level.data());
+      for (size_t jl = 0; jl <= nv; jl++) one.shift[jl] = one.lo[jl] ? (uint32_t)(nv - jl - h) : 0u;
+    }
     for (EqFactoring::One& one : ef.eqs) {
+      if (split) break;
       const Fr* shared = eq_half_lookup(c, one.y, num_vars, sharded);
       Fr* buf = c.arena.alloc_n<Fr>(shared ? half : 2 * half);
       one.level.resize(num_vars);
@@ -748,7 +778,7 @@
         }
         g.r = r;
         g.global_eq = -1;
-        g.eq_level = ef.eqs[0].level[round];
+        set_eq(g, round);
         g.pp = 1;
         k_sc_round(c, g, points, bind, size, out_host);
         ef.add_const = rw->const_total;
@@ -761,7 +791,7 @@
           g.lo[i] = out[2 * i], g.ro[i] = out[2 * i + 1];
           g.cs[i] = dev(rw->cs[i]), g.k[i] = dev(rw->k[i]);
         }
-        g.eq_level = ef.eqs[0].level[round];
+        set_eq(g, round);
         g.rchal = r;
         const bool fold = bind && c.opt.sc_pp_fold == 1;
         k_sc_round_rw(c, g, bind, size, out_host, fold);
@@ -800,7 +830,7 @@
         for (size_t i = 0; i < T; i++) g.in[i] = in[i], g.out[i] = out[i];
         g.r = r;
         g.global_eq = -1;
-        g.eq_level = ef.eqs[0].level[round];
+        set_eq(g, round);
         g.pp = pp_shape && points == 2 ? 1 : 0;
         if (g.pp && bind && pp_folded.empty() && c.opt.sc_pp_fold == 1) g.pp = 2;
         if (k_sc_round(c, g, points, bind, size, out_host)) {
@@ -892,7 +922,7 @@
         L.coef[m] = dev(co[m]), L.koff[m] = dev(ko[m]);
       }
       EqFactoring::One& e = ef.eqs[0];
-      L.eq_level = e.level[round];
+      L.eq_level = eq_level_full(c, e, num_vars, round);
       L.r_prev = dev(r_prev);
       std::vector<HFr> x, finals;
       if (!resident_tail_run(c, L, n0, e.y + round, ef.inv_1my.data() + round, e.S, ef.c, claim_now, rw ? rw->const_total : HFr::zero(),
diff --git a/include/lasso_hip.h b/include/lasso_hip.h
--- a/include/lasso_hip.h
+++ b/include/lasso_hip.h
@@ -177,7 +177,8 @@
   uint32_t resident_layers;
   uint32_t pp_folds;
   uint32_t msm_half_batches;
-  uint32_t reserved[7];
+  uint32_t eq_split_rounds;
+  uint32_t reserved[6];
 } lh_lasso_route;
 lh_status lh_lasso_last_route(lh_ctx*, lh_lasso_route* out);
 
```
